# willake/cpu-ray-tracer

Hardware: AMD Instinct MI355X
Metric: Mrays/sec (primary+secondary), 1280x720 64spp path trace — pipelined throughput over 878 consecutive 64-spp windows of one progressive render (single_render = one such render alone) (higher is better)
Workload: dtype f32; 1 GPU; bunny_scene.xml FileScene BVH-SAH path tracer, 1280x720, 64 spp/step (passes=1, depthLimit=5); 1 step = 64 frames = the next spp window of a progressive render; the 878 steps are one crt_render job (14 render kernel launch(es), a wavefront per (tile, 128 consecutive frames), + ordered accumulate), one sync at the end; triangles=4968, parallelism=tile-wave x1

## Files before the change

cpu-ray-tracer_amd/csrc/abi.cpp:

```cpp
#include "../../include/crt_abi.h"
#include "device/launch.h"
#include "host/grid_resolution.h"

#include <cmath>
#include <cstdarg>
#include <cstddef>
#include <cstdio>
#include <cstdlib>
#include <cstring>
#include <deque>
#include <string>
#include <algorithm>
#include <vector>
#include <chrono>

static_assert(sizeof(crt_bvh_node) == 32 && sizeof(crt_tri) == 112 && sizeof(crt_tlas_node) == 32, "reference layouts");
static_assert(sizeof(crt::NodePair) == 64 && sizeof(crt::LeafTri) == 48 && sizeof(crt::ShadeTri) == 64 && sizeof(crt::TlasNode) == 32 &&
              sizeof(crt::Instance) == 128 && sizeof(crt::Material) == 32 && offsetof(crt::Instance, T) == 64, "device layouts");
static_assert(sizeof(crt_counters) == sizeof(crt::Counters), "counter layout");
static_assert(sizeof(crt_kd_node) == 48 && sizeof(crt::KdNode) == sizeof(crt_kd_node) && sizeof(crt::AltTri) == 48, "flat KD node (uploaded as it comes), alternative accelerators' triangle record");
static_assert(offsetof(crt::PrimDev, red) == 536 && sizeof(crt::PrimDev) == 552, "PrimDev: 134 floats, then the two texel pointers");
static_assert(sizeof(crt::BlasAltDesc) == 72, "BLAS descriptor");
static_assert(sizeof(crt_shadow_ray) == 28 && sizeof(crt_ray) == 28 && sizeof(crt_hit) == 28, "query records");
static_assert(sizeof(crt_hit_info) == 48 && offsetof(crt_hit_info, material) == 12 && offsetof(crt_hit_info, N) == 16 && offsetof(crt_hit_info, albedo) == 32 && offsetof(crt_hit_info, v) == 44, "crt_hit_info: three 16-byte pieces");
// ... 221 lines not shown
}

}

extern "C" {

int crt_abi_version(void) { return CRT_ABI_VERSION; }

void crt_debug_enable_hooks(int on) { g_hooks = on != 0; }

int crt_device_count(void)
{
    int n = 0;
    if (hipGetDeviceCount(&n) != hipSuccess) return 0;
    return n;
}

const char* crt_last_error(crt_ctx* ctx) { return ctx ? ctx->err.c_str() : g_createError.c_str(); }

int crt_create(crt_ctx** out, const crt_config* cfg)
{
    if (!out || !cfg) { g_createError = "crt_create: null argument"; return CRT_ERR_INVALID; }
    *out = nullptr;
    setenv("GPU_MAX_HW_QUEUES", "16", 0);
    if (cfg->width < 16 || cfg->height < 16) { g_createError = "crt_create: width and height must be at least one 16x16 tile"; return CRT_ERR_INVALID; }
    int ndev = 0;
    hipError_t e = hipGetDeviceCount(&ndev);
    if (e != hipSuccess || ndev == 0) {
        g_createError = "crt_create: no HIP device visible (this library has no CPU path)";
        return CRT_ERR_NO_DEVICE;
    }
    if (cfg->device < 0 || cfg->device >= ndev) { g_createError = "crt_create: device ordinal out of range"; return CRT_ERR_INVALID; }
    crt_ctx* c = new crt_ctx();
    c->cfg = *cfg;
    if (const char* k = hook("CRT_RENDER_KERNEL")) {
        c->usePool = strcmp(k, "tiles") != 0;
        if (!strcmp(k, "pool_always")) c->poolMinWaves = 0;
    }
    if (c->cfg.depthLimit < 0) c->cfg.depthLimit = 5;
    if (c->cfg.depthLimit > 5) { g_createError = "crt_create: depthLimit > 5 unsupported (throughput stack holds 5 factors; reference default is 5)"; delete c; return CRT_ERR_UNSUPPORTED; }
    if (c->cfg.maxFramesPerLaunch <= 0) c->cfg.maxFramesPerLaunch = c->cfg.collectStats ? 64 : 4096;
    if (c->cfg.maxFramesPerLaunch > 64) c->cfg.maxFramesPerLaunch = c->cfg.maxFramesPerLaunch / 64 * 64;
    if (c->cfg.renderStreams < 0) c->cfg.renderStreams = 0;
    c->tilesX = cfg->width / 16; c->tilesY = cfg->height / 16;
    const int tiles = c->tilesX * c->tilesY;
    int first = cfg->tileFirst, stride = cfg->tileStride <= 0 ? 1 : cfg->tileStride, count = cfg->tileCount;
    if (count < 0) { first = 0; stride = 1; count = tiles; }
    if (first < 0 || (count > 0 && (long long)first + (long long)(count - 1) * stride >= tiles)) {
        g_createError = "crt_create: tile range exceeds the image"; delete c; return CRT_ERR_INVALID;
    }
    c->tileFirst = (uint32_t)first; c->tileStride = (uint32_t)stride; c->tileCount = (uint32_t)count;

    auto bail = [&](hipError_t he, const char* what) {
        g_createError = std::string("crt_create: ") + what + ": " + hipGetErrorString(he);
        crt_destroy(c); return CRT_ERR_DEVICE;
    };
    if ((e = hipSetDevice(cfg->device)) != hipSuccess) return bail(e, "hipSetDevice");
    if ((e = hipStreamCreateWithFlags(&c->stream, hipStreamNonBlocking)) != hipSuccess) return bail(e, "hipStreamCreate");
    const size_t px = (size_t)cfg->width * cfg->height;
    if ((e = hipMalloc(&c->dAccOwned, px * 16)) != hipSuccess) return bail(e, "hipMalloc(accumulator)");
    c->dAcc = c->dAccOwned;
    if ((e = hipMemsetAsync(c->dAcc, 0, px * 16, c->stream)) != hipSuccess) return bail(e, "hipMemset(accumulator)");
    if ((e = hipMalloc((void**)&c->dPixels, px * 4)) != hipSuccess) return bail(e, "hipMalloc(pixels)");
    if ((e = hipMemsetAsync(c->dPixels, 0, px * 4, c->stream)) != hipSuccess) return bail(e, "hipMemset(pixels)");
    if ((e = hipMalloc((void**)&c->dTileSums, (size_t)tiles * 4)) != hipSuccess) return bail(e, "hipMalloc(tileSums)");
    if ((e = hipMemsetAsync(c->dTileSums, 0, (size_t)tiles * 4, c->stream)) != hipSuccess) return bail(e, "hipMemset(tileSums)");
    if ((e = hipMalloc((void**)&c->dCounters, sizeof(crt::Counters))) != hipSuccess) return bail(e, "hipMalloc(counters)");
    if ((e = hipMemsetAsync(c->dCounters, 0, sizeof(crt::Counters), c->stream)) != hipSuccess) return bail(e, "hipMemset(counters)");
    if ((e = hipMalloc((void**)&c->dQueryCursor, 64)) != hipSuccess) return bail(e, "hipMalloc(query cursor)");
    if ((e = hipMalloc((void**)&c->dQuerySlots, crt_ctx::kQuerySlots * 64)) != hipSuccess) return bail(e, "hipMalloc(query cursor slots)");
    if (c->cfg.collectStats && count > 0) {
        if ((e = hipMalloc((void**)&c->dTileClocks, (size_t)count * 144)) != hipSuccess) return bail(e, "hipMalloc(tileClocks)");
        if ((e = hipMemsetAsync(c->dTileClocks, 0, (size_t)count * 144, c->stream)) != hipSuccess) return bail(e, "hipMemset(tileClocks)");
    }
    memset(&c->hScene, 0, sizeof(c->hScene));
    const float aspect = (float)cfg->width / (float)cfg->height;
    crt::Scene& s = c->hScene;
    s.camPos[0] = 0; s.camPos[1] = 0; s.camPos[2] = -2;
    s.topLeft[0] = -aspect; s.topLeft[1] = 1; s.topLeft[2] = 0;
    s.topRight[0] = aspect; s.topRight[1] = 1; s.topRight[2] = 0;
    s.bottomLeft[0] = -aspect; s.bottomLeft[1] = -1; s.bottomLeft[2] = 0;
    s.W = cfg->width; s.H = cfg->height; s.invW = 1.0f / cfg->width; s.invH = 1.0f / cfg->height;
    s.depthLimit = c->cfg.depthLimit;
    if ((e = hipStreamSynchronize(c->stream)) != hipSuccess) return bail(e, "hipStreamSynchronize");
    *out = c;
    return CRT_OK;
}

void crt_destroy(crt_ctx* c)
{
    if (!c) return;
    (void)hipSetDevice(c->cfg.device);
    for (auto st : c->streams) (void)hipStreamSynchronize(st);
    if (c->aheadStream) (void)hipStreamSynchronize(c->aheadStream);
    if (c->stream) (void)hipStreamSynchronize(c->stream);
    for (auto& q : c->qslot) if (q.done) { if (q.pending) (void)hipEventSynchronize(q.done); (void)hipEventDestroy(q.done); }
    if (c->dQuerySlots) (void)hipFree(c->dQuerySlots);
    if (c->altReady) (void)hipEventDestroy(c->altReady);
    if (c->writeFence) (void)hipEventDestroy(c->writeFence);
    c->refit.release(); c->tlasBuild.release();
    c->freeScene();
    c->gridBuild.release();
    for (hipEvent_t e : c->retiredEvents) (void)hipEventDestroy(e);
    for (auto& a : c->ahead) (void)hipEventDestroy(a.end);
    if (c->aheadStream) (void)hipStreamDestroy(c->aheadStream);
    for (auto& ev : c->evPool) { (void)hipEventDestroy(ev.a); (void)hipEventDestroy(ev.b); }
    for (auto& ev : c->evRender) { (void)hipEventDestroy(ev.a); (void)hipEventDestroy(ev.b); }
    for (auto& ev : c->evAcc) { (void)hipEventDestroy(ev.a); (void)hipEventDestroy(ev.b); }
    if (c->dAccOwned) (void)hipFree(c->dAccOwned);
    for (auto st : c->streams) { (void)hipStreamSynchronize(st); (void)hipStreamDestroy(st); }
    for (auto& r : c->inflight) (void)hipEventDestroy(r.freed);
    for (auto e : c->freeEvents) (void)hipEventDestroy(e);
    if (c->mustWait) (void)hipEventDestroy(c->mustWait);
    if (c->pool) (void)hipFree(c->pool);
    for (auto e : c->doneEvents) (void)hipEventDestroy(e);
    if (c->dPixels) (void)hipFree(c->dPixels);
    if (c->dTileSums) (void)hipFree(c->dTileSums);
    if (c->dCounters) (void)hipFree(c->dCounters);
    if (c->dQueryCursor) (void)hipFree(c->dQueryCursor);
    if (c->dInspectCounts) (void)hipFree(c->dInspectCounts);
    if (c->dInspectWork) (void)hipFree(c->dInspectWork);
    if (c->dTileClocks) (void)hipFree(c->dTileClocks);
    if (c->dTileOrder) (void)hipFree(c->dTileOrder);
    if (c->dTileCost) (void)hipFree(c->dTileCost);
    if (c->dJobCost) (void)hipFree(c->dJobCost);
    if (c->dJobDesc) (void)hipFree(c->dJobDesc);
    if (c->hJobDesc) (void)hipHostFree(c->hJobDesc);
    if (c->jobDescReady) (void)hipEventDestroy(c->jobDescReady);
    if (c->hJobCost) (void)hipHostFree(c->hJobCost);
    if (c->jobCostCopied) (void)hipEventDestroy(c->jobCostCopied);
    for (auto e : c->splitEvents) (void)hipEventDestroy(e);
    if (c->hTileCost) (void)hipHostFree(c->hTileCost);
    if (c->costCopied) (void)hipEventDestroy(c->costCopied);
    if (c->dBlockDesc) (void)hipFree(c->dBlockDesc);
    if (c->hBlockDesc) (void)hipHostFree(c->hBlockDesc);
    if (c->descReady) (void)hipEventDestroy(c->descReady);
    if (c->dStage) (void)hipFree(c->dStage);
    for (int k = 0; k < 2; k++) { if (c->hTileOrder[k]) (void)hipHostFree(c->hTileOrder[k]); if (c->orderCopied[k]) (void)hipEventDestroy(c->orderCopied[k]); }
    for (int k = 0; k < 2; k++) { if (c->hStage[k]) (void)hipHostFree(c->hStage[k]); if (c->stageCopied[k]) (void)hipEventDestroy(c->stageCopied[k]); }
    if (c->stream) (void)hipStreamDestroy(c->stream);
    delete c;
}

int crt_upload_scene(crt_ctx* c, const crt_scene_desc* sd)
{
    if (!c || !sd) return CRT_ERR_INVALID;
    c->epoch++;
    HIPCK(c, hipSetDevice(c->cfg.device));
    if (sd->kind != CRT_SCENE_FILE && sd->kind != CRT_SCENE_TLAS) return c->fail(CRT_ERR_INVALID, "unknown scene kind %d", sd->kind);
    if (!sd->bvhs || sd->bvhCount == 0) return c->fail(CRT_ERR_INVALID, "scene has no acceleration structure");
    if (sd->kind == CRT_SCENE_FILE && sd->bvhCount != 1) return c->fail(CRT_ERR_INVALID, "CRT_SCENE_FILE takes exactly one BVH (FileScene::acc)");
    if (sd->kind == CRT_SCENE_TLAS && (sd->bvhCount > 256 || !sd->tlasNodes || sd->tlasNodeCount < 2 * sd->bvhCount))
        return c->fail(CRT_ERR_INVALID, "TLAS scene needs <= 256 BLAS (tlas_bvh.cpp:21) and 2*blasCount TLAS nodes");
    if (sd->textureCount == 0 || !sd->textures) return c->fail(CRT_ERR_INVALID, "floor and skydome textures are required");
    if (sd->floorTexture < 0 || sd->floorTexture >= (int)sd->textureCount || sd->skyTexture < 0 || sd->skyTexture >= (int)sd->textureCount)
        return c->fail(CRT_ERR_INVALID, "floor/sky texture index out of range");
    for (uint32_t i = 0; i < sd->textureCount; i++)
        if (!sd->textures[i].pixels || sd->textures[i].width <= 0 || sd->textures[i].height <= 0) return c->fail(CRT_ERR_INVALID, "texture %u is empty", i);
    if (sd->materialCount > 0 && !sd->materials) return c->fail(CRT_ERR_INVALID, "materialCount is %u but materials is NULL", sd->materialCount);
    for (uint32_t i = 0; i < sd->materialCount; i++)
        if (sd->materials[i].texture >= (int)sd->textureCount) return c->fail(CRT_ERR_INVALID, "material %u: texture index out of range", i);
    if (sd->kind == CRT_SCENE_FILE) {
        if (!sd->objMatIdx || sd->objCount == 0) return c->fail(CRT_ERR_INVALID, "CRT_SCENE_FILE needs objMatIdx");
        for (uint32_t i = 0; i < sd->objCount; i++)
            if (sd->objMatIdx[i] < 0 || sd->objMatIdx[i] >= (int)sd->materialCount) return c->fail(CRT_ERR_INVALID, "objMatIdx entry out of range");
    }
// ... 127 lines not shown
        }
        tlasRoot = tlas[0].ref; tlasRoot16 = tlas[0].ref16;
    }
    std::vector<uint32_t> texOff(sd->textureCount); uint64_t texels = 0;
    for (uint32_t i = 0; i < sd->textureCount; i++) {
        texOff[i] = (uint32_t)texels;
        texels += (uint64_t)sd->textures[i].width * sd->textures[i].height;
        if (texels > 0xffffffffull) return c->fail(CRT_ERR_UNSUPPORTED, "texture pool exceeds 2^32 texels");
    }
    auto bindTex = [&](crt::Material& m, int t) {
        if (t < 0) { m.texOffset = 0; m.texW = 0; m.texH = 0; }
        else { m.texOffset = texOff[t]; m.texW = sd->textures[t].width; m.texH = sd->textures[t].height; }
    };
    std::vector<crt::Material> mats(2 + sd->materialCount);
    memset(mats.data(), 0, mats.size() * sizeof(crt::Material));
    bindTex(mats[0], -1);
    bindTex(mats[1], sd->floorTexture);
    for (uint32_t i = 0; i < sd->materialCount; i++) {
        crt::Material& m = mats[2 + i];
        m.reflectivity = sd->materials[i].reflectivity; m.refractivity = sd->materials[i].refractivity;
        memcpy(m.absorption, sd->materials[i].absorption, 12);
        bindTex(m, sd->materials[i].texture);
    }

    { const int r = drain_all(c); if (r) return r; }
    c->freeScene();
    uint32_t* dTexels = nullptr;
    HIPCK(c, hipMalloc((void**)&dTexels, (size_t)texels * 4)); c->sceneAllocs.push_back(dTexels);
    for (uint32_t i = 0; i < sd->textureCount; i++)
        HIPCK(c, hipMemcpyAsync(dTexels + texOff[i], sd->textures[i].pixels, (size_t)sd->textures[i].width * sd->textures[i].height * 4, hipMemcpyHostToDevice, c->stream));
    HIPCK(c, hipStreamSynchronize(c->stream));

    crt::Scene& s = c->hScene;
    s.kind = sd->kind;
    memcpy(s.lightInvT, sd->lightInvT, 48);
    s.lightNrm[0] = -sd->lightT[1]; s.lightNrm[1] = -sd->lightT[5]; s.lightNrm[2] = -sd->lightT[9];
    s.lightSize = sd->lightSize;
    {
        const float* m = sd->lightT;
        const float ax = -0.5f, ay = 0.0f, az = -0.5f, bx = 0.5f, by = 0.0f, bz = 0.5f;
        const float c1[3] = {m[0] * ax + m[1] * ay + m[2] * az + m[3] * 1.0f, m[4] * ax + m[5] * ay + m[6] * az + m[7] * 1.0f, m[8] * ax + m[9] * ay + m[10] * az + m[11] * 1.0f};
        const float c2[3] = {m[0] * bx + m[1] * by + m[2] * bz + m[3] * 1.0f, m[4] * bx + m[5] * by + m[6] * bz + m[7] * 1.0f, m[8] * bx + m[9] * by + m[10] * bz + m[11] * 1.0f};
        s.lightPos[0] = (c1[0] + c2[0]) * 0.5f - 0.0f; s.lightPos[1] = (c1[1] + c2[1]) * 0.5f - 0.01f; s.lightPos[2] = (c1[2] + c2[2]) * 0.5f - 0.0f;
    }
    memcpy(s.floorN, sd->floorN, 12); s.floorD = sd->floorD; s.floorInvto = sd->floorInvto;
    {
        const float* m = sd->lightInvT;
        s.lightAxis = (m[0] == 1.0f && m[1] == 0.0f && m[2] == 0.0f && m[4] == 0.0f && m[5] == 1.0f && m[6] == 0.0f && m[8] == 0.0f && m[9] == 0.0f && m[10] == 1.0f) ? 1u : 0u;
        s.floorAxisY = (sd->floorN[0] == 0.0f && sd->floorN[1] == 1.0f && sd->floorN[2] == 0.0f) ? 1u : 0u;
        if (hook("CRT_DEBUG_GENERAL_PRIMS")) s.lightAxis = s.floorAxisY = 0u;
    }
    s.floorMat = mats[1];
    s.skyOffset = texOff[sd->skyTexture]; s.skyW = sd->textures[sd->skyTexture].width; s.skyH = sd->textures[sd->skyTexture].height;
    s.texels = dTexels;
    int r;
    const char* dGeom = nullptr;
    if ((r = upload(c, geom, &dGeom))) return r;
    s.geom = dGeom;
    s.tlasOff = (uint32_t)tlasOffB; s.instOff = (uint32_t)instOffB; s.shadeOff = (uint32_t)shadeOffB;
    s.leafOff = (uint32_t)leafOffB; s.tlasPairOff = (uint32_t)tlasPairOffB;
    s.rootRef16 = (sd->kind == CRT_SCENE_TLAS) ? tlasRoot16 : rootRef0_16;
    s.ref16ok = (ref16ok && !hook("CRT_DEBUG_NO_REF16")) ? 1u : 0u;
    if ((r = upload(c, mats, &s.mats))) return r;
    if (sd->kind == CRT_SCENE_TLAS) {
        std::vector<float> boxes;
        for (uint32_t bi = 0; bi < sd->bvhCount; bi++) { const crt_bvh_node& n0 = sd->bvhs[bi].nodes[0]; boxes.insert(boxes.end(), n0.aabbMin, n0.aabbMin + 3); boxes.insert(boxes.end(), n0.aabbMax, n0.aabbMax + 3); }
        const float* d = nullptr;
        if ((r = upload(c, boxes, &d))) return r;
        c->dRootBox = const_cast<float*>(d);
    }
    s.rootRef = (sd->kind == CRT_SCENE_TLAS) ? tlasRoot : rootRef0;
    s.bvhStack = maxHeight > 0 ? maxHeight : 1;
    s.rootIsPair = 0; memset(s.rootPair, 0, sizeof(s.rootPair));
    if (sd->kind == CRT_SCENE_TLAS) {
        if ((tlasRoot & 0xC0000000u) == crt::kRefTlasInterior) {
            memcpy(s.rootPair, &tlas[tlasRoot & 0x7fffu], 32); memcpy(s.rootPair + 8, &tlas[(tlasRoot >> 15) & 0x7fffu], 32);
            s.rootIsPair = 1;
        }
    } else if (rootRef0 & crt::kRefInterior) {
        memcpy(s.rootPair, geom.data() + ((size_t)(rootRef0 & crt::kRefOffsetMask) << 4), 64);
        s.rootIsPair = 1;
    }
    if (hook("CRT_DEBUG_NO_ROOTPAIR")) s.rootIsPair = 0;
    s.stackDepth = s.bvhStack + ((sd->kind == CRT_SCENE_TLAS) ? tlasHeight + 1 : 0);
    c->ldsBytes = s.stackDepth * 64u * 4u; c->latSlots = 0;
    if (const char* e = hook("CRT_DEBUG_EXTRA_LDS")) c->ldsBytes += (uint32_t)atoi(e);
    if (c->ldsBytes + 15u * 256u > 64u * 1024u) return c->fail(CRT_ERR_UNSUPPORTED, "tree height %u (+TLAS %u) needs %u bytes of LDS traversal stack per wave (> 64 KiB)", maxHeight, tlasHeight, c->ldsBytes);
    {
        float lo[3] = {1e30f, 1e30f, 1e30f}, hi[3] = {-1e30f, -1e30f, -1e30f};
        auto grow = [&](const float* mn, const float* mx) { for (int k = 0; k < 3; k++) { if (mn[k] < lo[k]) lo[k] = mn[k]; if (mx[k] > hi[k]) hi[k] = mx[k]; } };
        if (sd->kind == CRT_SCENE_TLAS) grow(sd->tlasNodes[0].aabbMin, sd->tlasNodes[0].aabbMax);
        else grow(sd->bvhs[0].nodes[0].aabbMin, sd->bvhs[0].nodes[0].aabbMax);
        memcpy(c->meshLo, lo, 12); memcpy(c->meshHi, hi, 12); c->orderDirty = true;
    }
    {
        crt_ctx::Flat& f = c->flat;
        f.kind = sd->kind; f.leafOff = leafOffB; f.tlasOff = tlasOffB; f.tlasPairOff = tlasPairOffB; f.instOff = instOffB; f.shadeOff = shadeOffB;
        f.tlasNodeCount = (sd->kind == CRT_SCENE_TLAS) ? sd->tlasNodeCount : 0; f.maxHeight = maxHeight;
        f.objects = (sd->kind == CRT_SCENE_TLAS) ? sd->bvhCount : sd->objCount;
        f.pairBase.clear(); f.triBase.clear(); f.nodesUsed.clear(); f.triCount.clear(); f.rootBox.clear();
        for (uint32_t bi = 0; bi < sd->bvhCount; bi++) { const crt_bvh_node& r = sd->bvhs[bi].nodes[0]; f.rootBox.insert(f.rootBox.end(), r.aabbMin, r.aabbMin + 3); f.rootBox.insert(f.rootBox.end(), r.aabbMax, r.aabbMax + 3); }
        uint64_t pb = 0, tb = 0;
        for (uint32_t bi = 0; bi < sd->bvhCount; bi++) { f.pairBase.push_back(pb); f.triBase.push_back(tb); f.nodesUsed.push_back(sd->bvhs[bi].nodesUsed); f.triCount.push_back(sd->bvhs[bi].triCount); pb += sd->bvhs[bi].nodesUsed / 2; tb += sd->bvhs[bi].triCount; }
        f.geom.swap(geom);
    }
    c->haveScene = true;
    return CRT_OK;
}


static int order_behind_ahead(crt_ctx* c)
{
    for (const auto& a : c->ahead) HIPCK(c, hipStreamWaitEvent(c->stream, a.end, 0));
    return 0;
}

static int order_behind_queries(crt_ctx* c)
{
    for (auto& q : c->qslot) {
        if (!q.pending) continue;
        const hipError_t e = hipEventQuery(q.done);
        if (e == hipSuccess) { q.pending = false; continue; }
        if (e != hipErrorNotReady) return c->hip(e, "hipEventQuery(query)");
        HIPCK(c, hipStreamWaitEvent(c->stream, q.done, 0));
    }
    return 0;
}

static int wait_scene(crt_ctx* c, hipStream_t st)
{
    if (c->sceneReady) HIPCK(c, hipStreamWaitEvent(st, c->sceneReady, 0));
    return 0;
}

static int order_behind_readers(crt_ctx* c)
{
    int r;
    if ((r = order_behind_ahead(c)) || (r = order_behind_queries(c))) return r;
    c->epoch++;
    return 0;
}

static int begin_scene_write(crt_ctx* c, hipStream_t st)
{
    const int r = order_behind_readers(c);
    if (r || st == c->stream) return r;
    HIPCK(c, ensure_event(&c->writeFence));
    HIPCK(c, hipEventRecord(c->writeFence, c->stream));
    HIPCK(c, hipStreamWaitEvent(st, c->writeFence, 0));
    return wait_scene(c, st);
}

static int publish_scene_write(crt_ctx* c, hipStream_t st, hipEvent_t done)
{
    c->sceneReady = done;
    if (st != c->stream) HIPCK(c, hipStreamWaitEvent(c->stream, done, 0));
    return 0;
}

static int end_scene_write(crt_ctx* c, hipStream_t st, hipEvent_t done)
{
    HIPCK(c, hipEventRecord(done, st));
    return publish_scene_write(c, st, done);
}

static int flatten_tlas(crt_ctx* c, const crt_tlas_node* nodes, uint32_t count, uint32_t bvhCount, crt::TlasNode* tlas, crt::NodePair* tlasPairs, uint32_t* heightOut)
{
    uint32_t nTlasPairs = 0;
    for (uint32_t i = 0; i < count; i++) {
        const crt_tlas_node& nd = nodes[i];
        memcpy(tlas[i].lo, nd.aabbMin, 12); memcpy(tlas[i].hi, nd.aabbMax, 12);
        tlas[i].ref = nd.leftRight ? (crt::kRefTlasInterior | (nd.leftRight & 0x7fffu) | (((nd.leftRight >> 16) & 0x7fffu) << 15))
                                   : (crt::kRefTlasLeaf | (nd.BLAS & 0xffffu));
        tlas[i].ref16 = nd.leftRight ? (crt::kRef16TlasBit | nTlasPairs++) : (crt::kRef16TlasLeaf | (nd.BLAS & crt::kRef16IndexMask));
    }
    std::vector<std::pair<uint32_t, uint32_t>> st; st.push_back({0u, 0u}); size_t visited = 0; uint32_t height = 0;
    while (!st.empty()) {
        auto [n, d] = st.back(); st.pop_back();
        if (++visited > (size_t)count) return c->fail(CRT_ERR_INVALID, "TLAS node graph is not a tree");
        const crt_tlas_node& nd = nodes[n];
        if (nd.leftRight == 0) { if (nd.BLAS >= bvhCount) return c->fail(CRT_ERR_INVALID, "TLAS leaf references BLAS %u", nd.BLAS); if (d > height) height = d; continue; }
        const uint32_t l = nd.leftRight & 0xffffu, r = nd.leftRight >> 16;
        if (l >= count || r >= count) return c->fail(CRT_ERR_INVALID, "TLAS child index out of range");
        st.push_back({l, d + 1}); st.push_back({r, d + 1});
    }
    for (uint32_t i = 0; i < count; i++) {
        const crt_tlas_node& nd = nodes[i];
        if (nd.leftRight == 0) continue;
        crt::NodePair& p = tlasPairs[tlas[i].ref16 & crt::kRef16IndexMask];
        memcpy(&p.c[0], &tlas[nd.leftRight & 0xffffu], 32); memcpy(&p.c[1], &tlas[nd.leftRight >> 16], 32);
    }
    *heightOut = height;
    return 0;
}

static void set_root(crt_ctx* c, int kind, const float* lo, const float* hi)
{
    crt::Scene& s = c->hScene; const crt_ctx::Flat& f = c->flat;
    s.rootIsPair = 0; memset(s.rootPair, 0, sizeof(s.rootPair));
    if (kind == CRT_SCENE_TLAS) {
        const crt::TlasNode* tlas = reinterpret_cast<const crt::TlasNode*>(f.geom.data() + f.tlasOff);
        const uint32_t root = tlas[0].ref;
        s.rootRef = root; s.rootRef16 = tlas[0].ref16;
        if ((root & 0xC0000000u) == crt::kRefTlasInterior) { memcpy(s.rootPair, &tlas[root & 0x7fffu], 32); memcpy(s.rootPair + 8, &tlas[(root >> 15) & 0x7fffu], 32); s.rootIsPair = 1; }
    } else if (s.rootRef & crt::kRefInterior) {
        memcpy(s.rootPair, f.geom.data() + ((size_t)(s.rootRef & crt::kRefOffsetMask) << 4), 64);
        s.rootIsPair = 1;
    }
    if (hook("CRT_DEBUG_NO_ROOTPAIR")) s.rootIsPair = 0;
    memcpy(c->meshLo, lo, 12); memcpy(c->meshHi, hi, 12); c->orderDirty = true;
}

static int check_tlas_height(crt_ctx* c, uint32_t tlasHeight)
{
    if ((c->hScene.bvhStack + tlasHeight + 1) * 64u * 4u + 15u * 256u > 64u * 1024u)
        return c->fail(CRT_ERR_UNSUPPORTED, "TLAS height %u needs %u bytes of LDS traversal stack per wave (> 64 KiB)", tlasHeight, (c->hScene.bvhStack + tlasHeight + 1) * 256u);
    return 0;
}

static void adopt_tlas(crt_ctx* c, uint32_t tlasHeight, const float* lo, const float* hi)
{
    crt::Scene& s = c->hScene;
    s.stackDepth = s.bvhStack + tlasHeight + 1;
    c->ldsBytes = s.stackDepth * 64u * 4u; c->latSlots = 0;
    set_root(c, CRT_SCENE_TLAS, lo, hi);
}

static void drop_blas_sets(crt_ctx* c)
{
    for (int k = 0; k < 2; k++) if (c->haveBlas[k]) { c->haveBlas[k] = false; if (c->renderAccel == k + 1) c->renderAccel = 0; }
}

int crt_update_scene(crt_ctx* c, const crt_scene_desc* sd, uint32_t what)
{
    if (!c || !sd) return CRT_ERR_INVALID;
    if (!c->haveScene) return c->fail(CRT_ERR_STATE, "crt_update_scene before crt_upload_scene");
    crt_ctx::Flat& f = c->flat;
    if (sd->kind != f.kind || sd->bvhCount != f.nodesUsed.size() || !sd->bvhs) return c->fail(CRT_ERR_INVALID, "crt_update_scene: scene kind / BVH count differ from the uploaded scene");
    if ((what & ~(uint32_t)(CRT_UPDATE_TRANSFORMS | CRT_UPDATE_BOUNDS)) || what == 0) return c->fail(CRT_ERR_INVALID, "crt_update_scene: unknown update flags");
    if ((what & CRT_UPDATE_TRANSFORMS) && f.kind != CRT_SCENE_TLAS) return c->fail(CRT_ERR_INVALID, "CRT_UPDATE_TRANSFORMS applies to two-level scenes (a FileScene bakes its transforms into the triangles)");
    HIPCK(c, hipSetDevice(c->cfg.device));
    for (uint32_t bi = 0; bi < sd->bvhCount; bi++)
        if (sd->bvhs[bi].nodesUsed != f.nodesUsed[bi] || sd->bvhs[bi].triCount != f.triCount[bi] || !sd->bvhs[bi].nodes || !sd->bvhs[bi].triangles || !sd->bvhs[bi].triangleIndices)
            return c->fail(CRT_ERR_INVALID, "crt_update_scene: BVH %u changed its topology (node / triangle count); upload the scene again", bi);
    if (f.kind == CRT_SCENE_TLAS && (!sd->tlasNodes || sd->tlasNodeCount != f.tlasNodeCount))
        return c->fail(CRT_ERR_INVALID, "crt_update_scene: a two-level scene needs the node array of the TLASBVH::Build that followed the change (tlasNodes, %u nodes as uploaded)", f.tlasNodeCount);
    if (what & CRT_UPDATE_BOUNDS) {
        const crt::LeafTri* leaf = reinterpret_cast<const crt::LeafTri*>(f.geom.data() + f.leafOff);
        for (uint32_t bi = 0; bi < sd->bvhCount; bi++) {
            const crt_bvh& b = sd->bvhs[bi];
            for (uint32_t j = 0; j < b.triCount; j++) {
                const uint32_t ti = b.triangleIndices[j];
                if (ti >= b.triCount) return c->fail(CRT_ERR_INVALID, "BVH %u: triangleIndices[%u] out of range", bi, j);
                if (leaf[f.triBase[bi] + j].shadeIdx != (uint32_t)(f.triBase[bi] + ti)) return c->fail(CRT_ERR_INVALID, "BVH %u: triangleIndices changed; Refit keeps the leaf order — upload the scene again", bi);
            }
        }
    }
    uint32_t tlasHeight = 0;
    std::vector<char> tlasImage;
    if (f.kind == CRT_SCENE_TLAS) {
        tlasImage.assign((size_t)(f.instOff - f.tlasOff), 0);
        int r = flatten_tlas(c, sd->tlasNodes, sd->tlasNodeCount, sd->bvhCount, reinterpret_cast<crt::TlasNode*>(tlasImage.data()),
                             reinterpret_cast<crt::NodePair*>(tlasImage.data() + (f.tlasPairOff - f.tlasOff)), &tlasHeight);
        if (r || (r = check_tlas_height(c, tlasHeight))) return r;
    }
    size_t lo = SIZE_MAX, hi = 0;
    auto touch = [&](size_t a, size_t b) { if (a < lo) lo = a; if (b > hi) hi = b; };
    if (what & CRT_UPDATE_BOUNDS) {
        crt::NodePair* pairs = reinterpret_cast<crt::NodePair*>(f.geom.data());
        crt::LeafTri* leaf = reinterpret_cast<crt::LeafTri*>(f.geom.data() + f.leafOff);
        for (uint32_t bi = 0; bi < sd->bvhCount; bi++) {
            const crt_bvh& b = sd->bvhs[bi];
            for (uint32_t n = 1; n + 1 < b.nodesUsed; n += 2) {
                crt::NodePair& p = pairs[f.pairBase[bi] + ((n - 1) >> 1)];
                for (int k = 0; k < 2; k++) { memcpy(p.c[k].lo, b.nodes[n + k].aabbMin, 12); memcpy(p.c[k].hi, b.nodes[n + k].aabbMax, 12); }
            }
            for (uint32_t j = 0; j < b.triCount; j++) {
                const crt_tri& t = b.triangles[b.triangleIndices[j]];
                crt::LeafTri& lt = leaf[f.triBase[bi] + j];
                for (int k = 0; k < 3; k++) { lt.v0[k] = t.vertex0[k]; lt.e1[k] = t.vertex1[k] - t.vertex0[k]; lt.e2[k] = t.vertex2[k] - t.vertex0[k]; }
            }
        }
        touch(0, (size_t)f.tlasOff);
        for (uint32_t bi = 0; bi < sd->bvhCount; bi++) { memcpy(&f.rootBox[6 * bi], sd->bvhs[bi].nodes[0].aabbMin, 12); memcpy(&f.rootBox[6 * bi + 3], sd->bvhs[bi].nodes[0].aabbMax, 12); }
    }
    if (f.kind == CRT_SCENE_TLAS) {
        if (what & CRT_UPDATE_TRANSFORMS) {
            crt::Instance* inst = reinterpret_cast<crt::Instance*>(f.geom.data() + f.instOff);
            for (uint32_t bi = 0; bi < sd->bvhCount; bi++) { memcpy(inst[bi].invT, sd->bvhs[bi].invT, 48); memcpy(inst[bi].T, sd->bvhs[bi].T, 48); }
        }
        memcpy(f.geom.data() + f.tlasOff, tlasImage.data(), tlasImage.size());
        touch((size_t)f.tlasOff, (size_t)f.shadeOff);
    }
    if (lo >= hi) return CRT_OK;
    const int k = c->stageFlip ^= 1;
    const size_t boxBytes = ((what & CRT_UPDATE_BOUNDS) && c->dRootBox) ? f.rootBox.size() * 4u : 0u;
    const size_t geomBytes = hi - lo, bytes = geomBytes + boxBytes;
    if (c->stageBytes[k] < bytes) {
        if (c->hStage[k]) { HIPCK(c, hipEventSynchronize(c->stageCopied[k])); HIPCK(c, hipHostFree(c->hStage[k])); c->hStage[k] = nullptr; }
        HIPCK(c, hipHostMalloc((void**)&c->hStage[k], bytes, hipHostMallocDefault)); c->stageBytes[k] = bytes;
        HIPCK(c, ensure_event(&c->stageCopied[k]));
    } else HIPCK(c, hipEventSynchronize(c->stageCopied[k]));
    memcpy(c->hStage[k], f.geom.data() + lo, geomBytes);
    if (boxBytes) memcpy(c->hStage[k] + geomBytes, f.rootBox.data(), boxBytes);
    { const int r = begin_scene_write(c, c->stream); if (r) return r; }
    if (what & CRT_UPDATE_BOUNDS) {
        std::fill(c->blasGrid.current.begin(), c->blasGrid.current.end(), (uint8_t)0);
        drop_blas_sets(c);
    }
    HIPCK(c, hipMemcpyAsync(const_cast<char*>(c->hScene.geom) + lo, c->hStage[k], geomBytes, hipMemcpyHostToDevice, c->stream));
    if (boxBytes) HIPCK(c, hipMemcpyAsync(c->dRootBox, c->hStage[k] + geomBytes, boxBytes, hipMemcpyHostToDevice, c->stream));
    { const int r = end_scene_write(c, c->stream, c->stageCopied[k]); if (r) return r; }
    if (f.kind == CRT_SCENE_TLAS) adopt_tlas(c, tlasHeight, sd->tlasNodes[0].aabbMin, sd->tlasNodes[0].aabbMax);
    else set_root(c, f.kind, sd->bvhs[0].nodes[0].aabbMin, sd->bvhs[0].nodes[0].aabbMax);
    return CRT_OK;
}

int crt_set_camera(crt_ctx* c, const float camPos[3], const float tl[3], const float tr[3], const float bl[3])
{
    if (!c || !camPos || !tl || !tr || !bl) return CRT_ERR_INVALID;
    HIPCK(c, hipSetDevice(c->cfg.device));
    crt::Scene& s = c->hScene;
    if (!memcmp(s.camPos, camPos, 12) && !memcmp(s.topLeft, tl, 12) && !memcmp(s.topRight, tr, 12) && !memcmp(s.bottomLeft, bl, 12)) return CRT_OK;
    memcpy(s.camPos, camPos, 12); memcpy(s.topLeft, tl, 12); memcpy(s.topRight, tr, 12); memcpy(s.bottomLeft, bl, 12);
    c->orderDirty = true; c->epoch++;
    return CRT_OK;
}

static int upload_tile_order(crt_ctx* c, const std::vector<uint32_t>& order)
{
    if (!c->dTileOrder) HIPCK(c, hipMalloc((void**)&c->dTileOrder, (size_t)c->tileCount * 4));
    { const int r = order_behind_ahead(c); if (r) return r; }
    const int k = c->orderFlip ^= 1;
    if (!c->hTileOrder[k]) {
        HIPCK(c, hipHostMalloc((void**)&c->hTileOrder[k], (size_t)c->tileCount * 4, hipHostMallocDefault));
        HIPCK(c, ensure_event(&c->orderCopied[k]));
    } else HIPCK(c, hipEventSynchronize(c->orderCopied[k]));
    memcpy(c->hTileOrder[k], order.data(), order.size() * 4);
    HIPCK(c, hipMemcpyAsync(c->dTileOrder, c->hTileOrder[k], order.size() * 4, hipMemcpyHostToDevice, c->stream));
    HIPCK(c, hipEventRecord(c->orderCopied[k], c->stream));
    c->orderReady = c->orderCopied[k];
    return 0;
}

static int update_tile_order(crt_ctx* c)
{
    if (!c->orderDirty || c->tileCount == 0) return 0;
    const crt::Scene& s = c->hScene;
    double R[3], Dn[3], N[3];
    for (int k = 0; k < 3; k++) { R[k] = (double)s.topRight[k] - s.topLeft[k]; Dn[k] = (double)s.bottomLeft[k] - s.topLeft[k]; }
    N[0] = R[1] * Dn[2] - R[2] * Dn[1]; N[1] = R[2] * Dn[0] - R[0] * Dn[2]; N[2] = R[0] * Dn[1] - R[1] * Dn[0];
    const double rr = R[0] * R[0] + R[1] * R[1] + R[2] * R[2], dd = Dn[0] * Dn[0] + Dn[1] * Dn[1] + Dn[2] * Dn[2];
    double E[3]; for (int k = 0; k < 3; k++) E[k] = (double)s.topLeft[k] - s.camPos[k];
    const double num = E[0] * N[0] + E[1] * N[1] + E[2] * N[2];
    auto rect_of = [&](const float* P8, int r[4]) -> bool {
        double u0 = 1e30, u1 = -1e30, v0 = 1e30, v1 = -1e30;
        for (int i = 0; i < 8; i++) {
            const float* P = P8 + 3 * i;
            double d[3] = {P[0] - s.camPos[0], P[1] - s.camPos[1], P[2] - s.camPos[2]};
            const double den = d[0] * N[0] + d[1] * N[1] + d[2] * N[2];
            const double t = den != 0 ? num / den : -1;
            if (!(t > 0) || rr == 0 || dd == 0) return false;
            double Q[3]; for (int k = 0; k < 3; k++) Q[k] = s.camPos[k] + t * d[k] - s.topLeft[k];
            const double u = (Q[0] * R[0] + Q[1] * R[1] + Q[2] * R[2]) / rr, v = (Q[0] * Dn[0] + Q[1] * Dn[1] + Q[2] * Dn[2]) / dd;
            if (u < u0) u0 = u; if (u > u1) u1 = u; if (v < v0) v0 = v; if (v > v1) v1 = v;
        }
        r[0] = (int)floor(u0 * c->cfg.width / 16.0) - 1; r[1] = (int)floor(u1 * c->cfg.width / 16.0) + 1;
        r[2] = (int)floor(v0 * c->cfg.height / 16.0) - 1; r[3] = (int)floor(v1 * c->cfg.height / 16.0) + 1;
        return true;
    };
    float world[24];
    for (int i = 0; i < 8; i++) { world[3 * i] = (i & 1) ? c->meshHi[0] : c->meshLo[0]; world[3 * i + 1] = (i & 2) ? c->meshHi[1] : c->meshLo[1]; world[3 * i + 2] = (i & 4) ? c->meshHi[2] : c->meshLo[2]; }
    int wr[4] = {0, c->tilesX - 1, 0, c->tilesY - 1};
    (void)rect_of(world, wr);
    std::vector<uint32_t> first, second, rest;
    for (uint32_t i = 0; i < c->tileCount; i++) {
        const uint32_t tile = c->tileFirst + i * c->tileStride;
        const int tx = (int)(tile % (uint32_t)c->tilesX), ty = (int)(tile / (uint32_t)c->tilesX);
        const bool inRect = tx >= wr[0] && tx <= wr[1] && ty >= wr[2] && ty <= wr[3];
        if (inRect) first.push_back(i); else rest.push_back(i);
    }
    for (int k = 0; k <= crt_ctx::kLatStages; k++) { c->tuneCount[k] = 0; c->tuneMs[k] = 0; }
    c->latStage = 0; c->latBest = 0; c->latDone = false; c->latWarm = false; c->latConfirming = false; c->latQueue.clear(); c->costPending = false; c->latProbed = false;
    first.insert(first.end(), rest.begin(), rest.end());
    c->jobCostValid = false; c->jobCostPending = false; c->planValid = false;
    { const int r = upload_tile_order(c, first); if (r) return r; }
    c->orderDirty = false;
    return 0;
}

static size_t sample_bytes_per_window(const crt_ctx* c, uint32_t passes) { return (size_t)c->tileCount * 256u * 64u * passes * 16u; }
static size_t window_bytes(const crt_ctx* c, uint32_t passes) { return sample_bytes_per_window(c, passes) + (c->usePool ? crt_pool_scratch_bytes_per_window(c->tileCount) : 0); }

static uint32_t block_desc(uint32_t tile, uint32_t laneBase, uint32_t lanes, uint32_t window) { uint32_t lg = 0; while ((1u << lg) < lanes) lg++; return tile | (laneBase << 16) | (lg << 22) | (window << 25); }
static const uint32_t kLatLanes[7] = {64u, 32u, 16u, 8u, 4u, 2u, 1u};
static const double kLatG[7] = {1.0, 0.93, 0.88, 0.79, 0.69, 0.57, 0.48};
static int lat_index(uint32_t L) { int k = 0; while (k < 6 && kLatLanes[k] != L) k++; return k; }

static uint8_t next_lanes(uint8_t lanes, uint32_t cost, double T)
{
    int k = lat_index(lanes); const double unit = (double)cost / kLatG[k];
    while (k < 6 && unit * kLatG[k] > T) k++;
    while (k > 0 && unit * kLatG[k - 1] <= 0.9 * T) k--;
    return (uint8_t)kLatLanes[k];
}
extern "C" int crt_debug_next_lanes(const uint8_t* lanes, const uint32_t* cost, uint32_t n, double T, uint8_t* out)
{
// ... 1685 lines not shown
{
    if (!c || !out) return CRT_ERR_INVALID;
    int r;
    if ((r = sample_check(c, accel, 0, "crt_debug_sample_resident_lanes"))) return r;
    HIPCK(c, hipSetDevice(c->cfg.device));
    HIPCK(c, launch_sample(c, accel, nullptr, nullptr, nullptr, 0u, nullptr, out, c->stream));
    return CRT_OK;
}

int crt_get_light(crt_ctx* c, float pos[3], float color[3])
{
    if (!c || !pos || !color) return CRT_ERR_INVALID;
    if (!c->haveScene) return c->fail(c->havePrim ? CRT_ERR_UNSUPPORTED : CRT_ERR_STATE, "crt_get_light needs a triangle scene (crt_upload_scene)");
    memcpy(pos, c->hScene.lightPos, 12);
    color[0] = 24.0f; color[1] = 24.0f; color[2] = 22.0f;
    return CRT_OK;
}

int crt_get_counters(crt_ctx* c, crt_counters* out)
{
    if (!c || !out) return CRT_ERR_INVALID;
    HIPCK(c, hipSetDevice(c->cfg.device));
    HIPCK(c, hipMemcpyAsync(out, c->dCounters, sizeof(crt::Counters), hipMemcpyDeviceToHost, c->stream));
    HIPCK(c, hipStreamSynchronize(c->stream));
    return CRT_OK;
}

int crt_reset_counters(crt_ctx* c)
{
    if (!c) return CRT_ERR_INVALID;
    HIPCK(c, hipSetDevice(c->cfg.device));
    HIPCK(c, hipMemsetAsync(c->dCounters, 0, sizeof(crt::Counters), c->stream));
    return CRT_OK;
}

int crt_get_timing(crt_ctx* c, crt_timing* out)
{
    if (!c || !out) return CRT_ERR_INVALID;
    HIPCK(c, hipSetDevice(c->cfg.device));
    HIPCK(c, hipStreamSynchronize(c->stream));
    for (auto st : c->streams) HIPCK(c, hipStreamSynchronize(st));
    if (c->aheadStream) HIPCK(c, hipStreamSynchronize(c->aheadStream));
    harvest_tuning(c);
    memset(out, 0, sizeof(*out));
    out->render_kernel_ms = (float)c->foldedRenderMs; out->resolve_kernel_ms = (float)c->foldedAccMs;
    for (auto& ev : c->evRender) { float ms = 0; HIPCK(c, hipEventElapsedTime(&ms, ev.a, ev.b)); out->render_kernel_ms += ms; }
    for (auto& ev : c->evAcc) { float ms = 0; HIPCK(c, hipEventElapsedTime(&ms, ev.a, ev.b)); out->resolve_kernel_ms += ms; }
    out->render_launches = (uint32_t)c->evRender.size() + c->foldedLaunches;
    out->pool_launches = c->poolLaunches; out->split_launches = c->splitLaunches;
    c->foldedRenderMs = c->foldedAccMs = 0; c->foldedLaunches = 0; c->poolLaunches = 0; c->splitLaunches = 0;
    for (auto& ev : c->evRender) c->evPool.push_back(ev);
    for (auto& ev : c->evAcc) c->evPool.push_back(ev);
    c->evRender.clear(); c->evAcc.clear();
    return CRT_OK;
}

int crt_get_tile_clocks(crt_ctx* c, uint64_t* out)
{
    if (!c || !out) return CRT_ERR_INVALID;
    if (!c->dTileClocks) return c->fail(CRT_ERR_STATE, "tile clocks are recorded only by a collectStats context");
    HIPCK(c, hipSetDevice(c->cfg.device));
    HIPCK(c, hipMemcpyAsync(out, c->dTileClocks, (size_t)c->tileCount * 16, hipMemcpyDeviceToHost, c->stream));
    HIPCK(c, hipStreamSynchronize(c->stream));
    return CRT_OK;
}

extern "C" int crt_debug_live_events(crt_ctx* c) { return c ? (int)(2 * (c->evRender.size() + c->evAcc.size() + c->evPool.size())) : -1; }

extern "C" int crt_debug_check_reciprocals(crt_ctx* c, uint64_t* out)
{
    if (!c || !out) return CRT_ERR_INVALID;
    HIPCK(c, hipSetDevice(c->cfg.device));
    unsigned long long* d = nullptr;
    HIPCK(c, hipMalloc(&d, 32));
    hipError_t e = hipMemsetAsync(d, 0, 32, c->stream);
    if (e == hipSuccess) e = crt_launch_check_reciprocals(d, c->stream);
    if (e == hipSuccess) e = hipMemcpyAsync(out, d, 32, hipMemcpyDeviceToHost, c->stream);
    if (e == hipSuccess) e = hipStreamSynchronize(c->stream);
    (void)hipFree(d);
    HIPCK(c, e);
    return CRT_OK;
}

extern "C" int crt_debug_device_probe(crt_ctx* c, int op, const void* in, void* out, uint32_t n)
{
    static const uint8_t words[17][2] = {{1, 1}, {1, 1}, {2, 1}, {1, 1}, {2, 1}, {6, 7}, {1, 18}, {4, 1}, {5, 3}, {13, 2}, {16, 4}, {2, 2}, {2, 2}, {2, 2}, {2, 2}, {4, 2}, {2, 1}};
    if (!c || !in || !out || op < 0 || op > 16 || n > (1u << 25)) return CRT_ERR_INVALID;
    if (n == 0) return CRT_OK;
    const size_t inBytes = (size_t)n * words[op][0] * 4, outBytes = (size_t)n * words[op][1] * 4;
    HIPCK(c, hipSetDevice(c->cfg.device));
    char* d = nullptr;
    HIPCK(c, hipMalloc((void**)&d, inBytes + outBytes));
    hipError_t e = hipMemcpyAsync(d, in, inBytes, hipMemcpyHostToDevice, c->stream);
    if (e == hipSuccess) e = (op <= 10) ? crt_launch_probe_f32(op, d, d + inBytes, n, c->stream) : crt_launch_probe_f64(op, d, d + inBytes, n, c->stream);
    if (e == hipSuccess) e = hipMemcpyAsync(out, d + inBytes, outBytes, hipMemcpyDeviceToHost, c->stream);
    if (e == hipSuccess) e = hipStreamSynchronize(c->stream);
    (void)hipFree(d);
    HIPCK(c, e);
    return CRT_OK;
}

extern "C" int crt_debug_plan_job(const uint32_t* cost, uint32_t n, uint32_t windows, uint32_t frames, int pool, double poolWindowTicks,
                                  uint32_t* table, uint32_t tableCap, uint32_t* head, uint32_t* order)
{
    if (!cost || !n || !table || !head || !order) return CRT_ERR_INVALID;
    crt_ctx c;
    c.tileCount = n; c.jobCostValid = true; c.poolWindowTicks = poolWindowTicks;
    c.streams.assign(2, nullptr);
    c.jobCost.assign(cost, cost + n);
    c.jobOrder.resize(n);
    for (uint32_t i = 0; i < n; i++) c.jobOrder[i] = i;
    std::stable_sort(c.jobOrder.begin(), c.jobOrder.end(), [&](uint32_t a, uint32_t b) { return c.jobCost[a] > c.jobCost[b]; });
    std::vector<uint32_t> t; uint32_t h = 0;
    plan_job(&c, windows, frames, pool != 0, t, &h);
    c.streams.clear();
    if (t.size() > tableCap) return CRT_ERR_INVALID;
    memcpy(table, t.data(), t.size() * 4); memcpy(order, c.jobOrder.data(), (size_t)n * 4); *head = h;
    return (int)t.size();
}

extern "C" long long crt_debug_pool_wave_plan(const uint32_t* cost, uint32_t nr, uint32_t frames, double perCost, double startTicks, uint32_t resident, double safety, double guard,
                                              double share, uint32_t* wf, uint32_t* longFrames, double* start, double* aim)
{
    if (!nr || !frames || !wf || !longFrames) return CRT_ERR_INVALID;
    PoolWaveTerms tm; if (safety > 0) tm.safety = safety; if (guard > 0) tm.guard = guard; if (share > 0) tm.share = share;
    std::vector<uint32_t> w; std::vector<double> st;
    const uint64_t waves = pool_wave_plan(cost, nr, frames, crt_pool_streams(frames), perCost, startTicks, resident, tm, w, longFrames, &st, aim);
    memcpy(wf, w.data(), (size_t)nr * 4);
    if (start) memcpy(start, st.data(), (size_t)nr * 8);
    return (long long)waves;
}
extern "C" int crt_debug_pool_long_waves(crt_ctx* c) { return c ? (int)c->lastLongWaves : -1; }
extern "C" void crt_debug_pool_wave_terms(double* out) { const PoolWaveTerms tm; out[0] = tm.poolLong; out[1] = tm.load; out[2] = tm.safety; out[3] = tm.guard; out[4] = tm.share; }

extern "C" int crt_debug_tile_costs(crt_ctx* c, uint32_t* out)
{
    if (!c || !out || !c->dTileCost) return CRT_ERR_INVALID;
    HIPCK(c, hipSetDevice(c->cfg.device));
    HIPCK(c, hipDeviceSynchronize());
    HIPCK(c, hipMemcpy(out, c->dTileCost, (size_t)c->tileCount * 4, hipMemcpyDeviceToHost));
    return CRT_OK;
}

extern "C" int crt_debug_lat_stage(crt_ctx* c, int stage, uint8_t* lanes, uint32_t* cost)
{
    if (!c || stage < 0 || stage > crt_ctx::kLatStages) return CRT_ERR_INVALID;
    if (c->latL[stage].size() != c->tileCount || c->latCost[stage].size() != c->tileCount) return CRT_ERR_STATE;
    if (lanes) memcpy(lanes, c->latL[stage].data(), c->tileCount);
    if (cost) memcpy(cost, c->latCost[stage].data(), (size_t)c->tileCount * 4);
    return c->latStage;
}

extern "C" int crt_debug_tile_stamps(crt_ctx* c, uint64_t* out)
{
    if (!c || !out || !c->dTileClocks) return CRT_ERR_INVALID;
    HIPCK(c, hipSetDevice(c->cfg.device));
    HIPCK(c, hipMemcpyAsync(out, c->dTileClocks + 2 * (size_t)c->tileCount, (size_t)c->tileCount * 128, hipMemcpyDeviceToHost, c->stream));
    HIPCK(c, hipStreamSynchronize(c->stream));
    return CRT_OK;
}

int crt_bind_accumulator(crt_ctx* c, void* p)
{
    if (!c) return CRT_ERR_INVALID;
    if (p && ((uintptr_t)p & 15u)) return c->fail(CRT_ERR_INVALID, "accumulator pointer must be 16-byte aligned");
    HIPCK(c, hipSetDevice(c->cfg.device));
    HIPCK(c, hipStreamSynchronize(c->stream));
    c->dAcc = p ? p : c->dAccOwned;
    return CRT_OK;
}

int crt_accumulator_device_ptr(crt_ctx* c, void** p)
{
    if (!c || !p) return CRT_ERR_INVALID;
    *p = c->dAcc; return CRT_OK;
}

}
```

cpu-ray-tracer_amd/csrc/device/dev_common.h:

```cpp
#pragma once
#include <hip/hip_runtime.h>
#include <stddef.h>
#include <stdint.h>
#include "layout.h"

namespace crt {

struct f3 { float x, y, z; };
__device__ __forceinline__ f3 mk3(float x, float y, float z) { f3 r; r.x = x; r.y = y; r.z = z; return r; }
__device__ __forceinline__ f3 operator+(f3 a, f3 b) { return mk3(a.x + b.x, a.y + b.y, a.z + b.z); }
__device__ __forceinline__ f3 operator-(f3 a, f3 b) { return mk3(a.x - b.x, a.y - b.y, a.z - b.z); }
__device__ __forceinline__ f3 operator-(f3 a) { return mk3(-a.x, -a.y, -a.z); }
__device__ __forceinline__ f3 operator*(f3 a, f3 b) { return mk3(a.x * b.x, a.y * b.y, a.z * b.z); }
__device__ __forceinline__ f3 operator*(f3 a, float b) { return mk3(a.x * b, a.y * b, a.z * b); }
__device__ __forceinline__ f3 operator*(float b, f3 a) { return mk3(b * a.x, b * a.y, b * a.z); }
__device__ __forceinline__ float dot3(f3 a, f3 b) { return a.x * b.x + a.y * b.y + a.z * b.z; }
__device__ __forceinline__ f3 cross3(f3 a, f3 b) { return mk3(a.y * b.z - a.z * b.y, a.z * b.x - a.x * b.z, a.x * b.y - a.y * b.x); }
#ifdef CRT_IEEE_DIV
__device__ __forceinline__ float rcp_nr(float x) { return 1.0f / x; }
#else
__device__ __forceinline__ float rcp_nr(float x) { const float r = __builtin_amdgcn_rcpf(x); return __builtin_fmaf(__builtin_fmaf(-x, r, 1.0f), r, r); }
#endif
__device__ __forceinline__ float rcp_exact(float x)
{
    float r = rcp_nr(x);
    const float ax = __builtin_fabsf(x);
    if (__builtin_expect(__builtin_amdgcn_ballot_w64(!(ax >= 0x1p-126f && ax <= 0x1p126f)) != 0, 0)) r = 1.0f / x;
    return r;
}
__device__ __forceinline__ float rcp_exact_large(float x)
{
    float r = rcp_nr(x);
    if (__builtin_expect(__builtin_amdgcn_ballot_w64(!(__builtin_fabsf(x) <= 0x1p126f)) != 0, 0)) r = 1.0f / x;
    return r;
}
__device__ __forceinline__ f3 rcp_exact3(f3 v)
{
    f3 r = mk3(rcp_nr(v.x), rcp_nr(v.y), rcp_nr(v.z));
    const float ax = __builtin_fabsf(v.x), ay = __builtin_fabsf(v.y), az = __builtin_fabsf(v.z);
    const bool okay = ax >= 0x1p-126f && ay >= 0x1p-126f && az >= 0x1p-126f && ax <= 0x1p126f && ay <= 0x1p126f && az <= 0x1p126f;
    if (__builtin_expect(__builtin_amdgcn_ballot_w64(!okay) != 0, 0)) r = mk3(1.0f / v.x, 1.0f / v.y, 1.0f / v.z);
    return r;
}
__device__ __forceinline__ f3 normalize3(f3 v) { float inv = rcp_exact(__builtin_sqrtf(dot3(v, v))); return v * inv; }
__device__ __forceinline__ float min_std(float a, float b) { return (b < a) ? b : a; }
__device__ __forceinline__ float max_std(float a, float b) { return (a < b) ? b : a; }
__device__ __forceinline__ float min_tm(float a, float b) { return a < b ? a : b; }
__device__ __forceinline__ float max_tm(float a, float b) { return a > b ? a : b; }
__device__ __forceinline__ float clamp_tm(float f, float a, float b) { return max_tm(a, min_tm(f, b)); }
__device__ __forceinline__ int clampi(int f, int a, int b) { int m = (b < f) ? b : f; return (a < m) ? m : a; }
__device__ __forceinline__ float asf(uint32_t u) { return __uint_as_float(u); }
__device__ __forceinline__ uint32_t asu(float f) { return __float_as_uint(f); }

#define CRT_PI 3.14159265358979323846264f
#define CRT_INVPI 0.31830988618379067153777f
#define CRT_INV2PI 0.15915494309189533576888f
#define CRT_EPS 0.001f

static __device__ float crt_expf(float x)
{
    if (x != x) return x;
    if (x > 88.72283905206835f) return asf(0x7f800000u);
    if (x < -103.972084045410f) return 0.0f;
    float fk = __builtin_floorf(x * 1.44269504088896341f + 0.5f);
    float r = x - fk * 0.693359375f;
    r = r - fk * -2.12194440e-4f;
    float z = r * r;
    float p = 1.9875691500e-4f;
    p = p * r + 1.3981999507e-3f;
    p = p * r + 8.3334519073e-3f;
    p = p * r + 4.1665795894e-2f;
    p = p * r + 1.6666665459e-1f;
    p = p * r + 5.0000001201e-1f;
    p = p * z + r;
    p = p + 1.0f;
    int k = (int)fk;
    int k1 = k / 2, k2 = k - k1;
    float s1 = asf((uint32_t)(k1 + 127) << 23), s2 = asf((uint32_t)(k2 + 127) << 23);
    return p * s1 * s2;
}
__device__ __forceinline__ float crt_atan_pos(float x)
{
    const bool big = x > 2.414213562373095f, mid = x > 0.4142135623730950f;
    const float y0 = big ? 1.5707963267948966f : (mid ? 0.7853981633974483f : 0.0f);
    const float num = big ? -1.0f : (mid ? x - 1.0f : x);
    const float den = big ? x : (mid ? x + 1.0f : 1.0f);
    const float t = num / den;
    float z = t * t;
    float p = 8.05374449538e-2f;
    p = p * z - 1.38776856032e-1f;
    p = p * z + 1.99777106478e-1f;
    p = p * z - 3.33329491539e-1f;
    p = p * z * t + t;
    return y0 + p;
}
__device__ __forceinline__ float crt_atan2f(float y, float x)
{
    const uint32_t sy = asu(y) & 0x80000000u, sx = asu(x) & 0x80000000u;
    const float ax = __builtin_fabsf(x), ay = __builtin_fabsf(y);
    const float inf = asf(0x7f800000u);
    const float a = crt_atan_pos(ay / ax);
    float r = sx ? (CRT_PI - a) : a;
    if (ax == inf && ay == inf) r = sx ? 2.356194490192345f : 0.7853981633974483f;
    if (ax == 0.0f) r = 1.5707963267948966f;
    if (ay == 0.0f) r = sx ? CRT_PI : 0.0f;
    r = asf(asu(r) | sy);
    return (x != x || y != y) ? x + y : r;
}
__device__ __forceinline__ float crt_asin_small(float x)
{
    float z = x * x;
    float p = 4.2163199048e-2f;
    p = p * z + 2.4181311049e-2f;
    p = p * z + 4.5470025998e-2f;
    p = p * z + 7.4953002686e-2f;
    p = p * z + 1.6666752422e-1f;
    p = p * z * x + x;
    return p;
}
__device__ __forceinline__ float crt_acosf(float x)
{
    const bool hi = x > 0.5f, lo = x < -0.5f;
    const float s = __builtin_sqrtf(0.5f * (1.0f - __builtin_fabsf(x)));
    const float p = crt_asin_small((hi || lo) ? s : x);
    float r = hi ? 2.0f * p : (lo ? CRT_PI - 2.0f * p : 1.5707963267948966f - p);
    if (x > 1.0f || x < -1.0f) r = asf(0x7fc00000u);
    return (x != x) ? x : r;
}

__device__ __forceinline__ uint32_t wang_hash(uint32_t s)
{
    s = (s ^ 61u) ^ (s >> 16); s *= 9u; s = s ^ (s >> 4); s *= 0x27d4eb2du; s = s ^ (s >> 15); return s;
}
__device__ __forceinline__ uint32_t init_seed(uint32_t base) { return wang_hash((base + 1u) * 17u); }
__device__ __forceinline__ float rnd(uint32_t& s)
{
    s ^= s << 13; s ^= s >> 17; s ^= s << 5;
    return (float)s * 2.3283064365387e-10f;
}
__device__ __forceinline__ float rnd_pm1(uint32_t& s)
{
    s ^= s << 13; s ^= s >> 17; s ^= s << 5;
    return __builtin_fmaf((float)s, 4.656612873077392578125e-10f, -1.0f);
}


struct Hit { float t, u, v; int objIdx, triIdx; };
struct Cnt { uint32_t rays, primary, interior, leaf, tri, tlas, visits, meshhits; };

typedef float rec4 __attribute__((ext_vector_type(4)));
__device__ __forceinline__ rec4 ld4(const void* p) { return *reinterpret_cast<const rec4*>(p); }
__device__ __forceinline__ rec4 ldg(const char* __restrict__ base, uint32_t byteOff) { return *reinterpret_cast<const rec4*>(base + byteOff); }
__device__ __forceinline__ bool finite3(f3 v)
{
    const uint32_t m = 0x7f800000u;
    return ((asu(v.x) & m) != m) && ((asu(v.y) & m) != m) && ((asu(v.z) & m) != m);
}

__device__ __forceinline__ float box_exact(rec4 lo, rec4 hi, f3 O, f3 rD, float tray)
{
    float tx1 = (lo.x - O.x) * rD.x, tx2 = (hi.x - O.x) * rD.x;
    float tmin = min_std(tx1, tx2), tmax = max_std(tx1, tx2);
    float ty1 = (lo.y - O.y) * rD.y, ty2 = (hi.y - O.y) * rD.y;
    tmin = max_std(tmin, min_std(ty1, ty2)); tmax = min_std(tmax, max_std(ty1, ty2));
    float tz1 = (lo.z - O.z) * rD.z, tz2 = (hi.z - O.z) * rD.z;
    tmin = max_std(tmin, min_std(tz1, tz2)); tmax = min_std(tmax, max_std(tz1, tz2));
    return (tmax >= tmin && tmin < tray && tmax > 0) ? tmin : 1e30f;
}
__device__ __forceinline__ float vmin(float a, float b) { float r; asm("v_min_f32 %0, %1, %2" : "=v"(r) : "v"(a), "v"(b)); return r; }
__device__ __forceinline__ float vmax(float a, float b) { float r; asm("v_max_f32 %0, %1, %2" : "=v"(r) : "v"(a), "v"(b)); return r; }
__device__ __forceinline__ float vmin3(float a, float b, float c) { float r; asm("v_min3_f32 %0, %1, %2, %3" : "=v"(r) : "v"(a), "v"(b), "v"(c)); return r; }
__device__ __forceinline__ float vmax3(float a, float b, float c) { float r; asm("v_max3_f32 %0, %1, %2, %3" : "=v"(r) : "v"(a), "v"(b), "v"(c)); return r; }
__device__ __forceinline__ float box_fast(rec4 lo, rec4 hi, f3 O, f3 rD, float tray)
{
    float tx1 = (lo.x - O.x) * rD.x, tx2 = (hi.x - O.x) * rD.x;
    float ty1 = (lo.y - O.y) * rD.y, ty2 = (hi.y - O.y) * rD.y;
    float tz1 = (lo.z - O.z) * rD.z, tz2 = (hi.z - O.z) * rD.z;
    float tmin = vmax3(vmin(tx1, tx2), vmin(ty1, ty2), vmin(tz1, tz2));
    float tmax = vmin3(vmax(tx1, tx2), vmax(ty1, ty2), vmax(tz1, tz2));
    return (tmax >= tmin && tmin < tray && tmax > 0) ? tmin : 1e30f;
}

__device__ __forceinline__ void hit_tri(rec4 a, rec4 b, rec4 c, f3 O, f3 D, Hit& h)
{
    const f3 v0 = mk3(a.x, a.y, a.z), e1 = mk3(b.x, b.y, b.z), e2 = mk3(c.x, c.y, c.z);
    const f3 hh = cross3(D, e2);
    const float det = dot3(e1, hh);
    const float f = rcp_exact_large(det);
    const f3 s = O - v0;
    const float u = f * dot3(s, hh);
    const f3 q = cross3(s, e1);
    const float v = f * dot3(D, q);
    const float t = f * dot3(e2, q);
    const bool ok = !(det > -0.0001f && det < 0.0001f) && !(u < 0 || u > 1) && !(v < 0 || u + v > 1) && (t > 0.0001f) && (t < h.t);
    if (ok) { h.t = t; h.u = u; h.v = v; h.triIdx = (int)asu(a.w); h.objIdx = (int)asu(b.w); }
}

struct LightFloor { float lightInvT[12]; float lightSize; uint32_t lightAxis, floorAxisY; float floorN[3]; float floorD; };
__device__ __forceinline__ void hit_light_floor(const LightFloor& sc, f3 O, f3 D, Hit& h)
{
    {
        const float* c = sc.lightInvT;
        float Oy, Dy;
        if (sc.lightAxis) { Oy = O.y + c[7]; Dy = D.y; }
        else { Oy = c[4] * O.x + c[5] * O.y + c[6] * O.z + c[7]; Dy = c[4] * D.x + c[5] * D.y + c[6] * D.z; }
        const float t = Oy / -Dy;
        if (t < h.t && t > 0) {
            float Ox, Oz, Dx, Dz;
            if (sc.lightAxis) { Ox = O.x + c[3]; Oz = O.z + c[11]; Dx = D.x; Dz = D.z; }
            else {
                Ox = c[0] * O.x + c[1] * O.y + c[2] * O.z + c[3];
                Oz = c[8] * O.x + c[9] * O.y + c[10] * O.z + c[11];
                Dx = c[0] * D.x + c[1] * D.y + c[2] * D.z;
                Dz = c[8] * D.x + c[9] * D.y + c[10] * D.z;
            }
            const float Ix = Ox + t * Dx, Iz = Oz + t * Dz;
            const float size = sc.lightSize;
            if (Ix > -size && Ix < size && Iz > -size && Iz < size) { h.t = t; h.objIdx = 0; }
        }
    }
    {
        float num, den;
        if (sc.floorAxisY) { num = O.y + sc.floorD; den = D.y; }
        else { const f3 N = mk3(sc.floorN[0], sc.floorN[1], sc.floorN[2]); num = dot3(O, N) + sc.floorD; den = dot3(D, N); }
        const float t = -num / den;
        if (t < h.t && t > 0) { h.t = t; h.objIdx = 1; }
    }
}

__device__ __forceinline__ void hit_light_floor(const Scene& sc, f3 O, f3 D, Hit& h)
{
    LightFloor lf;
#pragma unroll
    for (int i = 0; i < 12; i++) lf.lightInvT[i] = sc.lightInvT[i];
    lf.lightSize = sc.lightSize; lf.lightAxis = sc.lightAxis; lf.floorAxisY = sc.floorAxisY;
    lf.floorN[0] = sc.floorN[0]; lf.floorN[1] = sc.floorN[1]; lf.floorN[2] = sc.floorN[2]; lf.floorD = sc.floorD;
    hit_light_floor(lf, O, D, h);
}

__device__ __forceinline__ bool quad_occluded(const Scene& sc, f3 O, f3 D, float tmax)
{
    const float* c = sc.lightInvT;
    const float Oy = c[4] * O.x + c[5] * O.y + c[6] * O.z + c[7];
    const float Dy = c[4] * D.x + c[5] * D.y + c[6] * D.z;
    const float t = Oy / -Dy;
    if (!(t < tmax && t > 0)) return false;
    const float Ox = c[0] * O.x + c[1] * O.y + c[2] * O.z + c[3];
    const float Oz = c[8] * O.x + c[9] * O.y + c[10] * O.z + c[11];
    const float Dx = c[0] * D.x + c[1] * D.y + c[2] * D.z;
    const float Dz = c[8] * D.x + c[9] * D.y + c[10] * D.z;
    const float Ix = Ox + t * Dx, Iz = Oz + t * Dz;
    const float size = sc.lightSize;
    return Ix > -size && Ix < size && Iz > -size && Iz < size;
}

static_assert(offsetof(Scene, topLeft) == offsetof(Scene, camPos) + 12 && offsetof(Scene, bottomLeft) == offsetof(Scene, camPos) + 36 && offsetof(Scene, invW) == offsetof(Scene, camPos) + 48 && offsetof(Scene, invH) == offsetof(Scene, camPos) + 52, "camera block");
static_assert(offsetof(Scene, lightSize) == offsetof(Scene, lightInvT) + 60 && offsetof(Scene, floorN) == offsetof(Scene, lightInvT) + 76 && offsetof(Scene, floorD) == offsetof(Scene, lightInvT) + 88 && offsetof(Scene, floorInvto) == offsetof(Scene, floorN) + 16, "light / floor block");
static_assert(offsetof(Scene, floorAxisY) == offsetof(Scene, lightAxis) + 4 && offsetof(Scene, skyW) == offsetof(Scene, skyOffset) + 4 && offsetof(Scene, skyH) == offsetof(Scene, skyOffset) + 8, "flag / sky words");
static_assert(offsetof(Material, absorption) == 8 && offsetof(Material, texOffset) == 20 && offsetof(Material, texW) == 24 && offsetof(Material, texH) == 28, "Material words");
typedef const float __attribute__((address_space(4)))* kernarg_f;
__device__ __forceinline__ kernarg_f scene_floats(size_t byteOffset)
{
    const char __attribute__((address_space(4)))* p = (const char __attribute__((address_space(4)))*)__builtin_amdgcn_kernarg_segment_ptr() + byteOffset;
    asm volatile("" : "+s"(p));
    return (kernarg_f)p;
}

__device__ __forceinline__ void to_object_space(rec4 r0, rec4 r1, rec4 r2, f3 O, f3 D, f3& Oo, f3& Do, f3& rDo)
{
    Oo = mk3((O.x * r0.x + O.y * r0.y) + (O.z * r0.z + 1.0f * r0.w),
             (O.x * r1.x + O.y * r1.y) + (O.z * r1.z + 1.0f * r1.w),
             (O.x * r2.x + O.y * r2.y) + (O.z * r2.z + 1.0f * r2.w));
    Do = mk3((D.x * r0.x + D.y * r0.y) + D.z * r0.z,
             (D.x * r1.x + D.y * r1.y) + D.z * r1.z,
             (D.x * r2.x + D.y * r2.y) + D.z * r2.z);
    rDo = rcp_exact3(Do);
}

__device__ __forceinline__ void traverse_bvh_seq(const Scene& sc, uint32_t rootRef, f3 O, f3 D, f3 rD, Hit& h, uint32_t* stk, Cnt& cn,
                                                 int& traversed, int& tested)
{
    const char* __restrict__ g = sc.geom;
    uint32_t cur = rootRef, sp = 0;
    for (;;) {
        traversed++;
        const uint32_t off = (cur & kRefOffsetMask) << 4;
        if (cur & kRefInterior) {
            cn.interior++;
            const rec4 alo = ldg(g, off), ahi = ldg(g, off + 16), blo = ldg(g, off + 32), bhi = ldg(g, off + 48);
            float d1 = box_exact(alo, ahi, O, rD, h.t), d2 = box_exact(blo, bhi, O, rD, h.t);
            uint32_t r1 = asu(alo.w), r2 = asu(blo.w);
            if (d1 > d2) { float td = d1; d1 = d2; d2 = td; uint32_t tr = r1; r1 = r2; r2 = tr; }
            if (d1 == 1e30f) { if (sp == 0) break; cur = stk[(--sp) * 64]; }
            else { cur = r1; if (d2 != 1e30f) { stk[sp * 64] = r2; sp++; } }
        } else {
            cn.leaf++;
            uint32_t o = off;
            for (;;) {
                const rec4 a = ldg(g, o), b = ldg(g, o + 16), c = ldg(g, o + 32);
                tested++; cn.tri++;
                hit_tri(a, b, c, O, D, h);
                if (asu(c.w) <= 1u) break;
                o += 48;
            }
            if (sp == 0) break;
            cur = stk[(--sp) * 64];
        }
    }
}

template <bool STOP = false, class BlasWalk>
__device__ __forceinline__ void tlas_walk(const Scene& sc, f3 O, f3 D, f3 rD, Hit& h, uint32_t* tstk, Cnt& cn, int& traversed, BlasWalk&& blas)
{
    const char* __restrict__ g = sc.geom;
    uint32_t cur = sc.rootRef, sp = 0;
    for (;;) {
        traversed++; cn.tlas++;
        if ((cur & kRefTlasLeaf) == kRefTlasLeaf) {
            cn.visits++;
            const uint32_t io = sc.instOff + (cur & 0xffffu) * 128u;
            const rec4 r0 = ldg(g, io), r1 = ldg(g, io + 16), r2 = ldg(g, io + 32), ids = ldg(g, io + 48);
            f3 Oo, Do, rDo; to_object_space(r0, r1, r2, O, D, Oo, Do, rDo);
            if constexpr (STOP) { if (blas(cur & 0xffffu, ids, Oo, Do, rDo)) break; }
            else blas(cur & 0xffffu, ids, Oo, Do, rDo);
            if (sp == 0) break;
            cur = tstk[(--sp) * 64];
        } else {
            const uint32_t o1 = sc.tlasOff + (cur & 0x7fffu) * 32u, o2 = sc.tlasOff + ((cur >> 15) & 0x7fffu) * 32u;
            const rec4 alo = ldg(g, o1), ahi = ldg(g, o1 + 16), blo = ldg(g, o2), bhi = ldg(g, o2 + 16);
            float d1 = box_exact(alo, ahi, O, rD, h.t), d2 = box_exact(blo, bhi, O, rD, h.t);
            uint32_t r1 = asu(alo.w), r2 = asu(blo.w);
            if (d1 > d2) { float td = d1; d1 = d2; d2 = td; uint32_t tr = r1; r1 = r2; r2 = tr; }
            if (d1 == 1e30f) { if (sp == 0) break; cur = tstk[(--sp) * 64]; }
            else { cur = r1; if (d2 != 1e30f) { tstk[sp * 64] = r2; sp++; } }
        }
    }
}

__device__ __forceinline__ void find_nearest_seq(const Scene& sc, f3 O, f3 D, f3 rD, Hit& h, uint32_t* stk, Cnt& cn, int& traversed, int& tested)
{
    cn.rays++;
    hit_light_floor(sc, O, D, h);
    if (sc.kind == 0) {
        traverse_bvh_seq(sc, sc.rootRef, O, D, rD, h, stk, cn, traversed, tested);
    } else {
        tlas_walk(sc, O, D, rD, h, stk + sc.bvhStack * 64, cn, traversed, [&](uint32_t, rec4 ids, f3 Oo, f3 Do, f3 rDo) __attribute__((always_inline)) {
            traverse_bvh_seq(sc, asu(ids.z), Oo, Do, rDo, h, stk, cn, traversed, tested);
        });
    }
    if (h.objIdx >= 2) cn.meshhits++;
}

__device__ __forceinline__ uint32_t tex_index(uint32_t offset, int w, int hgt, float u, float v)
{
    u = clamp_tm(u, 0.0f, 1.0f);
    v = 1 - clamp_tm(v, 0.0f, 1.0f);
    int x = (int)(u * w), y = (int)(v * hgt);
    x = clampi(x, 0, w - 1); y = clampi(y, 0, hgt - 1);
    return offset + (uint32_t)x + (uint32_t)y * (uint32_t)w;
}
__device__ __forceinline__ f3 tex_unpack(uint32_t p)
{
    const float s = 1 / 255.0f;
    return mk3(((p >> 16) & 0xFF) * s, ((p >> 8) & 0xFF) * s, (p & 0xFF) * s);
}
__device__ __forceinline__ f3 tex_sample(const Scene& sc, uint32_t offset, int w, int hgt, float u, float v)
{
    return tex_unpack(sc.texels[tex_index(offset, w, hgt, u, v)]);
}

__device__ __forceinline__ f3 sky_color(const Scene& sc, f3 D)
{
    float phi = crt_atan2f(-D.z, D.x) + CRT_PI;
    float theta = crt_acosf(-D.y);
    return tex_sample(sc, sc.skyOffset, sc.skyW, sc.skyH, phi * CRT_INV2PI, theta * CRT_INVPI);
}

__device__ __forceinline__ uint32_t wave_sum(uint32_t v)
{
    for (int o = 32; o > 0; o >>= 1) v += __shfl_xor(v, o, 64);
    return v;
}

}
```

cpu-ray-tracer_amd/csrc/device/kernels.hip:

```cpp
#include "alt_common.h"
#include "launch.h"

namespace crt {

#ifndef CRT_SHADE_BATCH
#define CRT_SHADE_BATCH 24
#endif
#ifndef CRT_SHADE_BATCH_JOB
#define CRT_SHADE_BATCH_JOB 40
#endif
#ifndef CRT_TRI_BATCH
#define CRT_TRI_BATCH 1
#endif
#ifndef CRT_NODE_BATCH
#define CRT_NODE_BATCH 1
#endif

#ifndef CRT_TILES_NODE_STEPS
#define CRT_TILES_NODE_STEPS 2
#endif
#ifndef CRT_MIN_WAVES
#define CRT_MIN_WAVES 5
#endif
template <int KIND, bool COUNT>
// ... 939 lines not shown
    const int32_t before = __shfl_up(incl, 1, 64);
    if (lane > 0 && before > peak) peak = before;
    if (idx < n && pixels[idx] == kInspectPending) {
        const f3 res = traverse_count_color(own, peak);
        acc[idx] = make_float4(res.x, res.y, res.z, 0.0f);
        const uint32_t r = (uint32_t)(255.0f * min_std(1.0f, res.x)), g = (uint32_t)(255.0f * min_std(1.0f, res.y)), bb = (uint32_t)(255.0f * min_std(1.0f, res.z));
        pixels[idx] = (r << 16) + (g << 8) + bb;
    }
}

__global__ __launch_bounds__(64) void resolve_kernel(const float4* __restrict__ acc, uint32_t* __restrict__ pixels, float* __restrict__ tileSums,
                                                      uint32_t tileFirst, uint32_t tileStride, uint32_t tileCount, uint32_t tilesX,
                                                      uint32_t W, float scale)
{
    const uint32_t tl = blockIdx.x * blockDim.x + threadIdx.x;
    if (tl >= tileCount) return;
    const uint32_t tile = tileFirst + tl * tileStride;
    const uint32_t x0 = (tile % tilesX) * 16u, y0 = (tile / tilesX) * 16u;
    float sum = 0;
    for (uint32_t v = 0; v < 16; v++) for (uint32_t u = 0; u < 16; u++) {
        const size_t i = (x0 + u) + (size_t)(y0 + v) * W;
        const float4 a = acc[i];
        const float px = a.x * scale, py = a.y * scale, pz = a.z * scale;
        sum += px + py + pz;
        const uint32_t r = (uint32_t)(255.0f * min_std(1.0f, px)), g = (uint32_t)(255.0f * min_std(1.0f, py)), bb = (uint32_t)(255.0f * min_std(1.0f, pz));
        pixels[i] = (r << 16) + (g << 8) + bb;
    }
    tileSums[tile] = sum;
}

__global__ __launch_bounds__(256) void commit_frame_kernel(const float4* __restrict__ slabWindow, uint32_t frameInWindow, uint32_t passes,
                                                            float4* __restrict__ acc, uint32_t* __restrict__ pixels, float* __restrict__ tileSums,
                                                            uint32_t tileFirst, uint32_t tileStride, uint32_t tileCount, uint32_t tilesX,
                                                            uint32_t W, float scale)
{
    __shared__ float tileE[256];
    const uint32_t tl = blockIdx.x, pix = threadIdx.x;
    if (tl >= tileCount) return;
    const uint32_t tile = tileFirst + tl * tileStride;
    const uint32_t x0 = (tile % tilesX) * 16u, y0 = (tile / tilesX) * 16u;
    const size_t i = (x0 + (pix & 15u)) + (size_t)(y0 + (pix >> 4)) * W;
    const float4* __restrict__ s = slabWindow + ((size_t)tl * 256u + pix) * (64u * passes) + frameInWindow * passes;
    float4 a = acc[i];
    for (uint32_t p = 0; p < passes; p++) { const float4 t = s[p]; a.x += t.x; a.y += t.y; a.z += t.z; a.w += t.w; }
    acc[i] = a;
    const float px = a.x * scale, py = a.y * scale, pz = a.z * scale;
    tileE[pix] = px + py + pz;
    const uint32_t r = (uint32_t)(255.0f * min_std(1.0f, px)), g = (uint32_t)(255.0f * min_std(1.0f, py)), bb = (uint32_t)(255.0f * min_std(1.0f, pz));
    pixels[i] = (r << 16) + (g << 8) + bb;
    __syncthreads();
    if (pix == 0) {
        float sum = 0;
        for (uint32_t k = 0; k < 256u; k++) sum += tileE[k];
        tileSums[tile] = sum;
    }
}

}

namespace crt {
__device__ __forceinline__ bool same_bits(float a, float b) { return asu(a) == asu(b) || (a != a && b != b); }
__global__ __launch_bounds__(256) void check_reciprocals_kernel(unsigned long long* out)
{
    const uint32_t tid = blockIdx.x * 256u + threadIdx.x, nthreads = gridDim.x * 256u;
    unsigned long long n = 0, bad1 = 0, bad2 = 0, bad3 = 0;
    for (uint64_t b = tid; b < (1ull << 32); b += nthreads) {
        const float x = asf((uint32_t)b), want = 1.0f / x;
        n++;
        if (!same_bits(rcp_exact(x), want)) bad1++;
        if (!(__builtin_fabsf(x) < 0.0001f) && !same_bits(rcp_exact_large(x), want)) bad2++;
        const float y = asf((uint32_t)b * 2654435761u), z = asf(((uint32_t)b >> 7) * 40503u + 0x3f000000u);
        const f3 r = rcp_exact3(mk3(x, y, z));
        if (!same_bits(r.x, want) || !same_bits(r.y, 1.0f / y) || !same_bits(r.z, 1.0f / z)) bad3++;
    }
    atomicAdd(&out[0], n); atomicAdd(&out[1], bad1); atomicAdd(&out[2], bad2); atomicAdd(&out[3], bad3);
}
}
extern "C" hipError_t crt_launch_check_reciprocals(unsigned long long* out, hipStream_t stream)
{
    hipLaunchKernelGGL(crt::check_reciprocals_kernel, dim3(4096), dim3(256), 0, stream, out);
    return hipGetLastError();
}

extern "C" hipError_t crt_launch_render(const crt::Scene* sc, void* slab, crt::Counters* counters, unsigned long long* tileClocks, const uint32_t* tileOrder,
                                        uint32_t tileFirst, uint32_t tileStride, uint32_t tileCount, uint32_t tilesX, uint32_t sppFirst,
                                        uint32_t frames, uint32_t passes, uint32_t ldsBytes, int collectStats, const uint32_t* blockDesc, uint32_t nBlocks, uint32_t* tileCost, uint32_t rankCount, unsigned long long* launchClk, hipStream_t stream)
{
    if (tileCount == 0 || frames == 0) return hipSuccess;
    const uint32_t windows = (frames + 63u) / 64u;
    if ((unsigned long long)tileCount * windows > 0x7fffffffull) return hipErrorInvalidValue;
    if (collectStats || nBlocks == 0u) blockDesc = nullptr;
    if (blockDesc && (tileCount > 0x10000u || windows > 64u)) return hipErrorInvalidValue;
    if (rankCount == 0u || rankCount > tileCount) rankCount = tileCount;
    dim3 grid(blockDesc ? nBlocks : rankCount * windows), block(64);
#define CRT_LAUNCH(K, C) hipLaunchKernelGGL((crt::render_tiles_kernel<K, C>), grid, block, ldsBytes + 15u * 64u * 4u , stream, *sc, (float4*)slab, counters, tileClocks, tileOrder, tileFirst, tileStride, tileCount, tilesX, sppFirst, frames, passes, windows, blockDesc, tileCost, rankCount, launchClk)
    if (sc->kind == 0) { if (collectStats) CRT_LAUNCH(0, true); else CRT_LAUNCH(0, false); }
    else { if (collectStats) CRT_LAUNCH(1, true); else CRT_LAUNCH(1, false); }
#undef CRT_LAUNCH
    return hipGetLastError();
}

extern "C" uint32_t crt_render_resident_waves(int device, int kind, uint32_t ldsBytes)
{
    int perCu = 0, cus = 0;
    const size_t lds = (size_t)ldsBytes + 15u * 64u * 4u;
    hipError_t e = kind == 0 ? hipOccupancyMaxActiveBlocksPerMultiprocessor(&perCu, crt::render_tiles_kernel<0, false>, 64, lds)
                             : hipOccupancyMaxActiveBlocksPerMultiprocessor(&perCu, crt::render_tiles_kernel<1, false>, 64, lds);
    if (e != hipSuccess || hipDeviceGetAttribute(&cus, hipDeviceAttributeMultiprocessorCount, device) != hipSuccess || perCu <= 0 || cus <= 0) { (void)hipGetLastError(); return 5120u; }
    return (uint32_t)perCu * (uint32_t)cus;
}

extern "C" hipError_t crt_launch_accumulate(const void* slab, void* acc, uint32_t tileFirst, uint32_t tileStride, uint32_t tileCount,
                                            uint32_t tilesX, uint32_t W, uint32_t frames, uint32_t passes, hipStream_t stream)
{
    if (tileCount == 0 || frames == 0) return hipSuccess;
    dim3 grid(tileCount), block(256);
    hipLaunchKernelGGL(crt::accumulate_kernel, grid, block, 4u * crt::kAccWaveLds, stream, (const float4*)slab, (float*)acc, tileFirst, tileStride, tileCount, tilesX, W, frames, passes);
    return hipGetLastError();
}

extern "C" hipError_t crt_launch_find_nearest(const crt::Scene* sc, const void* rays, void* hits, uint32_t n, crt::Counters* counters,
                                              uint32_t ldsBytes, uint32_t* cursor, hipStream_t stream)
{
    hipError_t e; if (!crt::query_launch_begin(n, cursor, stream, &e)) return e;
    dim3 grid(crt::query_grid(n, ldsBytes)), block(64);
    hipLaunchKernelGGL(crt::find_nearest_kernel, grid, block, ldsBytes, stream, *sc, (const crt::RayIn*)rays, (crt::HitOut*)hits, n, counters, cursor);
    return hipGetLastError();
}

extern "C" hipError_t crt_launch_is_occluded(const crt::Scene* sc, const void* rays, int32_t* occluded, uint32_t n, uint32_t ldsBytes, uint32_t* cursor, hipStream_t stream)
{
    hipError_t e; if (!crt::query_launch_begin(n, cursor, stream, &e)) return e;
    dim3 grid(crt::query_grid(n, ldsBytes)), block(64);
    hipLaunchKernelGGL(crt::is_occluded_kernel, grid, block, ldsBytes, stream, *sc, (const crt::ShadowRayIn*)rays, occluded, n, cursor);
    return hipGetLastError();
}

extern "C" hipError_t crt_launch_whitted(const crt::Scene* sc, int accel, const crt::AltAccelDev* alt, const crt::TlasAltDev* tl, void* acc, uint32_t* pixels, crt::Counters* counters, uint32_t ldsBytes,
                                         hipStream_t stream)
{
    const uint32_t n = (uint32_t)sc->W * (uint32_t)sc->H;
    dim3 grid((n + 63u) / 64u), block(64);
    if (accel != 0 && sc->kind != 0) {
        const uint32_t bytes = crt::tlas_alt_stack_words(*sc, *tl) * 64u * 4u;
        if (bytes > 64u * 1024u) return hipErrorInvalidValue;
        if (accel == 1) hipLaunchKernelGGL((crt::whitted_kernel<1, crt::TlasAltDev>), grid, block, bytes, stream, *sc, *tl, (float4*)acc, pixels, counters);
        else hipLaunchKernelGGL((crt::whitted_kernel<2, crt::TlasAltDev>), grid, block, bytes, stream, *sc, *tl, (float4*)acc, pixels, counters);
        return hipGetLastError();
    }
    if (accel == 1) hipLaunchKernelGGL(crt::whitted_kernel<1>, grid, block, alt->kdStack * 128u * 4u, stream, *sc, *alt, (float4*)acc, pixels, counters);
    else if (accel == 2) hipLaunchKernelGGL(crt::whitted_kernel<2>, grid, block, 256u, stream, *sc, *alt, (float4*)acc, pixels, counters);
    else { const crt::AltAccelDev none{}; hipLaunchKernelGGL(crt::whitted_kernel<0>, grid, block, ldsBytes, stream, *sc, none, (float4*)acc, pixels, counters); }
    return hipGetLastError();
}

template <int ACCEL, class ALT>
static hipError_t launch_whitted_inspect(const crt::Scene& sc, const ALT& alt, uint32_t ldsBytes, int inspect, int32_t peakIn, float4* acc, uint32_t* pixels, crt::Counters* counters,
                                         int32_t* trav, int32_t* tested, crt::InspectSums* sums, int32_t* blockMax, hipStream_t stream)
{
    const uint32_t n = (uint32_t)sc.W * (uint32_t)sc.H;
    dim3 grid((n + 63u) / 64u), block(64);
    if (inspect == 0) {
        const crt::InspectOut out{trav, tested, sums};
        hipLaunchKernelGGL((crt::whitted_kernel<ACCEL, ALT, crt::InspectOut>), grid, block, ldsBytes, stream, sc, alt, acc, pixels, counters, out);
        return hipGetLastError();
    }
// ... 52 lines not shown
```

cpu-ray-tracer_amd/csrc/device/launch.h:

```cpp
#pragma once
#include "layout.h"

#include <hip/hip_runtime.h>

extern "C" {

hipError_t crt_launch_check_reciprocals(unsigned long long* out, hipStream_t stream);
hipError_t crt_launch_render(const crt::Scene* sc, void* slab, crt::Counters* counters, unsigned long long* tileClocks, const uint32_t* tileOrder, uint32_t tileFirst, uint32_t tileStride,
    uint32_t tileCount, uint32_t tilesX, uint32_t sppFirst, uint32_t frames, uint32_t passes, uint32_t ldsBytes, int collectStats, const uint32_t* blockDesc, uint32_t nBlocks, uint32_t* tileCost,
    uint32_t rankCount, unsigned long long* launchClk, hipStream_t stream);
uint32_t crt_render_resident_waves(int device, int kind, uint32_t ldsBytes);
hipError_t crt_launch_accumulate(const void* slab, void* acc, uint32_t tileFirst, uint32_t tileStride, uint32_t tileCount, uint32_t tilesX, uint32_t W, uint32_t frames, uint32_t passes,
    hipStream_t stream);
hipError_t crt_launch_find_nearest(const crt::Scene* sc, const void* rays, void* hits, uint32_t n, crt::Counters* counters, uint32_t ldsBytes, uint32_t* cursor, hipStream_t stream);
hipError_t crt_launch_is_occluded(const crt::Scene* sc, const void* rays, int32_t* occluded, uint32_t n, uint32_t ldsBytes, uint32_t* cursor, hipStream_t stream);
hipError_t crt_launch_whitted(const crt::Scene* sc, int accel, const crt::AltAccelDev* alt, const crt::TlasAltDev* tl, void* acc, uint32_t* pixels, crt::Counters* counters, uint32_t ldsBytes,
    hipStream_t stream);
size_t crt_whitted_inspect_work_bytes(uint32_t pixelCount);
hipError_t crt_launch_whitted_inspect(const crt::Scene* sc, int accel, const crt::AltAccelDev* alt, const crt::TlasAltDev* tl, int inspect, int32_t peakIn, void* acc, uint32_t* pixels,
    crt::Counters* counters, int32_t* trav, int32_t* tested, void* work, uint32_t ldsBytes, hipStream_t stream);
hipError_t crt_launch_resolve(const void* acc, uint32_t* pixels, float* tileSums, uint32_t tileFirst, uint32_t tileStride, uint32_t tileCount, uint32_t tilesX, uint32_t W, float scale,
    hipStream_t stream);
hipError_t crt_launch_commit_frame(const void* slabWindow, uint32_t frameInWindow, uint32_t passes, void* acc, uint32_t* pixels, float* tileSums, uint32_t tileFirst, uint32_t tileStride,
    uint32_t tileCount, uint32_t tilesX, uint32_t W, float scale, hipStream_t stream);

uint32_t crt_pool_streams(uint32_t frames);
size_t crt_pool_scratch_bytes_per_window(uint32_t tileCount);
hipError_t crt_launch_render_pool(const crt::Scene* sc, void* slab, void* facScratch, crt::Counters* counters, unsigned long long* tileClocks, const uint32_t* tileOrder, uint32_t tileFirst,
    uint32_t tileStride, uint32_t tileCount, uint32_t tilesX, uint32_t sppFirst, uint32_t frames, uint32_t passes, int collectStats, uint32_t rankFirst, uint32_t waveFrames,
    const uint32_t* waveTab, uint32_t tabBlocks, uint32_t longFrames, uint32_t* tileCost, unsigned long long* launchClk, hipStream_t stream);
uint32_t crt_pool_lds_bytes(uint32_t stackDepth, uint32_t streams);
int crt_debug_pool_stamps(unsigned long long* out, int reset);
int crt_debug_pool_density(unsigned long long* out, int reset);
size_t crt_debug_pool_timeline(unsigned long long* out, size_t cap);

uint32_t crt_probe_paths(void);
hipError_t crt_launch_probe(const crt::Scene* sc, uint32_t tileFirst, uint32_t tileStride, uint32_t tileCount, uint32_t tilesX, uint32_t* tileCost, hipStream_t stream);
hipError_t crt_launch_render_alt(int accel, const crt::Scene* sc, const crt::AltAccelDev* acc, const crt::TlasAltDev* tl, void* slab, crt::Counters* counters, uint32_t tileFirst, uint32_t tileStride,
    uint32_t tileCount, uint32_t tilesX, uint32_t sppFirst, uint32_t frames, uint32_t passes, hipStream_t stream);
hipError_t crt_launch_sample_query(int accel, const crt::Scene* sc, const crt::AltAccelDev* acc, const crt::TlasAltDev* tl, const void* rays, uint32_t* seeds, float* rgb, uint32_t n,
    crt::Counters* counters, uint32_t* cursor, uint32_t* residentLanes, hipStream_t stream);

hipError_t crt_launch_find_nearest_prim(const crt::PrimDev* p, const void* rays, void* hits, uint32_t n, hipStream_t stream);
hipError_t crt_launch_render_prim(const crt::Scene* sc, const crt::PrimDev* p, void* slab, crt::Counters* counters, uint32_t tileFirst, uint32_t tileStride, uint32_t tileCount, uint32_t tilesX,
    uint32_t sppFirst, uint32_t frames, uint32_t passes, hipStream_t stream);
hipError_t crt_launch_sample_query_prim(const crt::Scene* sc, const crt::PrimDev* p, const void* rays, uint32_t* seeds, float* rgb, uint32_t n, crt::Counters* counters, uint32_t* cursor,
    uint32_t* residentLanes, hipStream_t stream);
hipError_t crt_launch_probe_f64(int op, const void* in, void* out, uint32_t n, hipStream_t stream);

hipError_t crt_launch_find_nearest_alt(int kind, const crt::Scene* sc, const crt::AltAccelDev* acc, const void* rays, void* hits, uint32_t n, uint32_t* cursor, hipStream_t stream);
hipError_t crt_launch_is_occluded_alt(int kind, const crt::Scene* sc, const crt::AltAccelDev* acc, const void* rays, int32_t* occluded, uint32_t n, uint32_t* cursor, hipStream_t stream);
hipError_t crt_launch_tlas_alt_query(int kind, bool occl, const crt::Scene* sc, const crt::TlasAltDev* tl, const void* rays, void* out, uint32_t n, uint32_t* cursor, hipStream_t stream);

hipError_t crt_launch_hit_info(const crt::Scene* sc, const void* rays, const void* hits, void* out, uint32_t n, uint32_t objects, uint32_t fileTris, hipStream_t stream);
hipError_t crt_launch_sky_color(const crt::Scene* sc, const void* rays, float* rgb, uint32_t n, hipStream_t stream);
hipError_t crt_launch_refit(char* geom, uint32_t leafOff, uint32_t pairBase, uint32_t triBase, uint32_t triCount, const float* pos, const void* plan, const uint32_t* levelOff, uint32_t levels,
    uint32_t rootCode, float* out, hipStream_t stream);
hipError_t crt_launch_probe_f32(int op, const void* in, void* out, uint32_t n, hipStream_t stream);

uint32_t crt_grid_build_blocks(int device);
size_t crt_grid_scan_chunks(uint32_t cells);
hipError_t crt_launch_grid_bounds(const float* pos, uint32_t triCount, crt::GridBuildState* state, uint32_t maxBlocks, hipStream_t stream);
hipError_t crt_launch_grid_count(const float* pos, uint32_t triCount, const crt::GridParams* g, uint32_t cells, uint32_t* counts, unsigned long long* chunkSums, crt::GridBuildState* state,
    uint32_t maxBlocks, hipStream_t stream);
hipError_t crt_launch_grid_fill(const float* pos, uint32_t triCount, const crt::GridParams* g, uint32_t cells, const uint32_t* cellStart, uint32_t* cursor, int32_t* unsorted, int32_t* refs,
    uint32_t total, const char* geom, uint32_t leafOff, uint32_t triBase, int globalIdx, crt::AltTri* tris, uint32_t maxBlocks, hipStream_t stream);

hipError_t crt_launch_tlas_build(const char* geom, uint32_t instOff, const float* T, const float* rootBox, uint32_t blasCount, uint32_t pairRel, uint32_t instRel, void* out,
    hipStream_t stream);

uint32_t crt_debug_query_grid(void);

}

namespace crt {

inline uint32_t bounded_query_grid(uint32_t grid) { const uint32_t k = crt_debug_query_grid(); return (k != 0u && k < grid) ? k : grid; }

inline uint32_t query_grid(uint32_t n, uint32_t ldsBytes)
{
    uint32_t perCu = ldsBytes ? (160u * 1024u) / ldsBytes : 16u; if (perCu > 16u) perCu = 16u; if (perCu < 4u) perCu = 4u;
    const uint32_t need = (n + 63u) / 64u, fill = 256u * perCu;
    return bounded_query_grid(need < fill ? need : fill);
}

inline bool query_launch_begin(uint32_t n, uint32_t* cursor, hipStream_t stream, hipError_t* status)
{
    *status = hipSuccess;
    if (n == 0) return false;
    if (!cursor) { *status = hipErrorInvalidValue; return false; }
// ... 6 lines not shown
```

cpu-ray-tracer_amd/csrc/device/layout.h:

```cpp
#pragma once
#include <stdint.h>

namespace crt {

constexpr uint32_t kRefInterior = 0x80000000u;
constexpr uint32_t kRefTlasBit = 0x40000000u;
constexpr uint32_t kRefTlasInterior = 0x40000000u;
constexpr uint32_t kRefTlasLeaf = 0xC0000000u;
constexpr uint32_t kRefReturn = 0xFFFFFFFFu;
constexpr uint32_t kRefDone = 0u;
constexpr uint32_t kRefOffsetMask = 0x3fffffffu;
constexpr uint64_t kMaxGeomBytes = 1ull << 32;

constexpr uint32_t kRef16Interior = 0x8000u, kRef16TlasBit = 0x4000u, kRef16TlasLeaf = 0xC000u, kRef16TagMask = 0xC000u, kRef16IndexMask = 0x3fffu;
constexpr uint32_t kRef16Return = 0xFFFFu, kRef16MaxIndex = 0x3ffeu;

struct alignas(16) NodeChild { float lo[3]; uint32_t ref; float hi[3]; uint32_t ref16; };
struct alignas(64) NodePair { NodeChild c[2]; };

struct alignas(16) LeafTri {
    float v0[3]; uint32_t shadeIdx;
    float e1[3]; int32_t objIdx;
    float e2[3]; uint32_t remain;
};

struct alignas(16) ShadeTri {
    float n0[3], n1[3], n2[3];
    float uv0[2], uv1[2], uv2[2];
    int32_t mat;
};

struct alignas(16) TlasNode { float lo[3]; uint32_t ref; float hi[3]; uint32_t ref16; };

struct alignas(16) Instance {
    float invT[12];
    uint32_t shadeBase;
    uint32_t rootRef16;
    uint32_t rootRef;
    int32_t objIdx;
    float T[12];
    uint32_t triCount;
    uint32_t pad[3];
};

struct alignas(16) Material {
    float reflectivity, refractivity;
    float absorption[3];
    uint32_t texOffset;
    int32_t texW, texH;
};

struct Scene {
    int32_t kind;
    int32_t depthLimit;
    float camPos[3], topLeft[3], topRight[3], bottomLeft[3];
    float invW, invH;
    int32_t W, H;
    float lightInvT[12]; float lightNrm[3]; float lightSize;
    float lightPos[3];
    float floorN[3]; float floorD; float floorInvto;
    Material floorMat;
    uint32_t skyOffset; int32_t skyW, skyH;
    const char* geom;
    uint32_t tlasOff, instOff, shadeOff;
    uint32_t leafOff, tlasPairOff;
    uint32_t rootRef16, ref16ok;
    const uint32_t* texels;
    const Material* mats;
    uint32_t rootRef;
    uint32_t stackDepth;
    uint32_t bvhStack;
    uint32_t lightAxis, floorAxisY;
    uint32_t rootIsPair;
    float rootPair[16];
};

struct Counters { unsigned long long v[8]; };

struct alignas(16) RefitPlanRec { uint32_t pair, child[2], pad; };
constexpr uint32_t kPlanInterior = 0x80000000u;

struct alignas(64) TlasBuildHeader {
    uint32_t status;
    uint32_t step;
    uint32_t height;
    uint32_t searches;
    uint32_t staleA;
    uint32_t pad[11];
};
constexpr uint32_t kTlasBuildOk = 0u, kTlasBuildNoCandidate = 1u, kTlasBuildNoEnd = 2u;
constexpr uint32_t kTlasMaxBlas = 256u;

#if defined(__HIPCC__)
#define CRT_HOST_DEVICE __host__ __device__
#else
#define CRT_HOST_DEVICE
#endif
template <class TriCountOf>
CRT_HOST_DEVICE inline bool hit_record_ok(int32_t objIdx, int32_t triIdx, uint32_t objects, TriCountOf&& triCountOf)
{
    if (objIdx < 2) return objIdx >= -1;
    if ((uint32_t)(objIdx - 2) >= objects) return false;
    return triIdx >= 0 && (uint32_t)triIdx < triCountOf((uint32_t)(objIdx - 2));
}

struct KdNode { float lo[3]; int32_t left; float hi[3]; int32_t right; float splitDistance; int32_t splitAxis; uint32_t firstTri, triCount; };
struct AltTri { float v0[3]; uint32_t triIdx; float e1[3]; int32_t objIdx; float e2[3]; uint32_t pad; };
struct AltAccelDev {
    const KdNode* kdNodes; const uint32_t* kdRefs; uint32_t kdStack;
    const AltTri* tris;
    int32_t res[3]; float cell[3]; float lo[3], hi[3]; const uint32_t* cellStart; const int32_t* cellRefs;
};

struct BlasAltDesc {
    uint32_t nodeBase, refBase, triBase;
    uint32_t cellBase, cellRefBase;
    int32_t objIdx;
    int32_t res[3]; float cell[3]; float lo[3], hi[3];
};
struct TlasAltDev {
    const BlasAltDesc* desc;
    const void* kdNodes; const uint32_t* kdRefs; const void* tris;
    const uint32_t* cellStart; const int32_t* cellRefs;
    uint32_t kdStack;
};

struct GridParams { int32_t res[3]; float cell[3]; float lo[3]; };
struct alignas(16) GridBuildState { unsigned long long key[6]; unsigned long long total; uint32_t nonFinite; uint32_t pad; };

struct PrimDev {
    float quadInvT[12], quadNrm[3], quadSize;
    float spherePos[3], pad0;
    float cubeInvM[12], cubeM[12], cubeMin[3], cubeMax[3];
    float torusInvT[12], torusT[12], rt2, rc2, r2, pad1;
    float refl[11], refr[11], absorb[33];
    float pad2;
    const uint32_t* red; const uint32_t* blue;
};

}
```

cpu-ray-tracer_amd/csrc/device/probe.hip:

```cpp
#include "dev_common.h"
#include "launch.h"

namespace crt {

__global__ __launch_bounds__(256) void probe_f32_kernel(int op, const uint32_t* __restrict__ in, uint32_t* __restrict__ out, uint32_t n)
{
    const uint32_t i = blockIdx.x * 256u + threadIdx.x;
    if (i >= n) return;
    switch (op) {
    case 0: out[i] = asu(crt_expf(asf(in[i]))); break;
    case 1: out[i] = asu(crt_acosf(asf(in[i]))); break;
    case 2: out[i] = asu(crt_atan2f(asf(in[2 * (size_t)i]), asf(in[2 * (size_t)i + 1]))); break;
    case 3: out[i] = asu(__builtin_sqrtf(asf(in[i]))); break;
    case 4: out[i] = asu(asf(in[2 * (size_t)i]) / asf(in[2 * (size_t)i + 1])); break;
    case 5: {
        const uint32_t* p = in + 6 * (size_t)i; uint32_t* o = out + 7 * (size_t)i;
        const f3 a = mk3(asf(p[0]), asf(p[1]), asf(p[2])), b = mk3(asf(p[3]), asf(p[4]), asf(p[5]));
        const f3 nn = normalize3(a), cr = cross3(a, b);
        o[0] = asu(nn.x); o[1] = asu(nn.y); o[2] = asu(nn.z); o[3] = asu(cr.x); o[4] = asu(cr.y); o[5] = asu(cr.z); o[6] = asu(dot3(a, b));
        break;
    }
    case 6: {
        uint32_t* o = out + 18 * (size_t)i;
        uint32_t s = init_seed(in[i]);
        o[0] = s;
#pragma unroll
        for (int k = 0; k < 8; k++) o[1 + k] = asu(rnd(s));
#pragma unroll
        for (int k = 0; k < 8; k++) o[9 + k] = asu(rnd_pm1(s));
        o[17] = s;
        break;
    }
    case 7: {
        const uint32_t* p = in + 4 * (size_t)i;
        out[i] = tex_index(0u, (int)p[2], (int)p[3], asf(p[0]), asf(p[1]));
        break;
    }
    case 8: {
        const uint32_t* p = in + 5 * (size_t)i; uint32_t* o = out + 3 * (size_t)i;
        const f3 D = mk3(asf(p[0]), asf(p[1]), asf(p[2]));
        const float phi = crt_atan2f(-D.z, D.x) + CRT_PI;
        const float theta = crt_acosf(-D.y);
        o[0] = asu(phi); o[1] = asu(theta); o[2] = tex_index(0u, (int)p[3], (int)p[4], phi * CRT_INV2PI, theta * CRT_INVPI);
        break;
    }
    case 9: {
        const uint32_t* p = in + 13 * (size_t)i;
        rec4 lo, hi; lo.x = asf(p[0]); lo.y = asf(p[1]); lo.z = asf(p[2]); lo.w = 0.0f; hi.x = asf(p[3]); hi.y = asf(p[4]); hi.z = asf(p[5]); hi.w = 0.0f;
        const f3 O = mk3(asf(p[6]), asf(p[7]), asf(p[8])), rD = mk3(asf(p[9]), asf(p[10]), asf(p[11]));
        const float tray = asf(p[12]);
        out[2 * (size_t)i] = asu(box_exact(lo, hi, O, rD, tray)); out[2 * (size_t)i + 1] = asu(box_fast(lo, hi, O, rD, tray));
        break;
    }
    case 10: {
        const uint32_t* p = in + 16 * (size_t)i; uint32_t* o = out + 4 * (size_t)i;
        rec4 a, b, c;
        a.x = asf(p[0]); a.y = asf(p[1]); a.z = asf(p[2]); a.w = asf(7u);
        b.x = asf(p[3]); b.y = asf(p[4]); b.z = asf(p[5]); b.w = asf(2u);
        c.x = asf(p[6]); c.y = asf(p[7]); c.z = asf(p[8]); c.w = asf(1u);
        const f3 O = mk3(asf(p[9]), asf(p[10]), asf(p[11])), D = mk3(asf(p[12]), asf(p[13]), asf(p[14]));
        Hit h; h.t = asf(p[15]); h.u = 0.0f; h.v = 0.0f; h.objIdx = -1; h.triIdx = -1;
        hit_tri(a, b, c, O, D, h);
        o[0] = asu(h.t); o[1] = asu(h.u); o[2] = asu(h.v); o[3] = (h.triIdx == 7) ? 1u : 0u;
        break;
    }
    default: break;
    }
}

}

extern "C" hipError_t crt_launch_probe_f32(int op, const void* in, void* out, uint32_t n, hipStream_t stream)
{
    if (n == 0) return hipSuccess;
    if (op < 0 || op > 10) return hipErrorInvalidValue;
    hipLaunchKernelGGL(crt::probe_f32_kernel, dim3((n + 255u) / 256u), dim3(256), 0, stream, op, (const uint32_t*)in, (uint32_t*)out, n);
    return hipGetLastError();
}
```

cpu-ray-tracer_amd/csrc/device/render_pool.hip:

```cpp
#include "dev_common.h"
#include "launch.h"

namespace crt {

enum : uint32_t {
    F_OX = 0, F_OY, F_OZ, F_DX, F_DY, F_DZ,
    F_RX, F_RY, F_RZ,
    F_T,
    F_SEED, F_META,
    F_U, F_V,
    F_COUNT,
    F_CUR = F_U, F_PEND = F_V,
    F_TRI = F_RX
};
constexpr uint32_t kMetaItemMask = 0x7ffu, kMetaDepthShift = 11u, kMetaInside = 1u << 14, kMetaFresh = 1u << 15, kMetaObjShift = 16u, kMetaLowMask = 0xffffu;
constexpr uint32_t kQueueMask = 127u;

#ifndef CRT_POOL_MIN_WAVES
#define CRT_POOL_MIN_WAVES 4
#endif
#ifndef CRT_POOL_SHADE_MIN
#define CRT_POOL_SHADE_MIN 64
#endif
#ifndef CRT_POOL_NODE_STEPS
#define CRT_POOL_NODE_STEPS 2
#endif
#ifndef CRT_POOL_NODE2_MIN
#define CRT_POOL_NODE2_MIN 16
#endif
#ifndef CRT_POOL_STARVE
#define CRT_POOL_STARVE 40
#endif

#ifdef CRT_POOL_STAMPS
__device__ unsigned long long g_poolStamps[16];
#define CRT_PSTAMP(var) unsigned long long var; asm volatile("s_memtime %0\n\ts_waitcnt lgkmcnt(0)" : "=s"(var) :: "memory")
#define CRT_PACC(i, a, b) (pst[i] += (b) - (a))
#else
#define CRT_PSTAMP(var)
#define CRT_PACC(i, a, b)
#endif
#ifdef CRT_POOL_DENS
__device__ unsigned long long g_poolDens[48];
#define CRT_DENS(i, v) (dens[i] += (uint32_t)(v))
#define CRT_DENS_MASK(i, pred) (dens[i] += (uint32_t)__popcll(__builtin_amdgcn_ballot_w64(pred)))
#define CRT_LIVE_BUCKET(n) ((n) >= 112u ? 0u : (n) >= 96u ? 1u : (n) >= 64u ? 2u : 3u)
#else
#define CRT_DENS(i, v)
#define CRT_DENS_MASK(i, pred)
#endif
#ifdef CRT_POOL_TIMELINE
__device__ unsigned long long* g_poolTimeline = nullptr;
#endif
__device__ __forceinline__ bool lane_in(uint64_t m) { return __builtin_amdgcn_inverse_ballot_w64(m); }
__device__ __forceinline__ uint64_t finite3_mask(f3 v)
{
    const uint32_t m = 0x7f800000u;
    return __builtin_amdgcn_ballot_w64((asu(v.x) & m) != m) & __builtin_amdgcn_ballot_w64((asu(v.y) & m) != m) & __builtin_amdgcn_ballot_w64((asu(v.z) & m) != m);
}
__device__ __forceinline__ uint32_t rank_in(uint64_t m) { return __builtin_amdgcn_mbcnt_hi((uint32_t)(m >> 32), __builtin_amdgcn_mbcnt_lo((uint32_t)m, 0u)); }

template <int KIND, bool COUNT, int S>
__global__ __launch_bounds__(64, CRT_POOL_MIN_WAVES) void render_pool_kernel(const Scene sc, float4* __restrict__ slab, float* __restrict__ facScratch, Counters* __restrict__ counters,
                                                             unsigned long long* __restrict__ tileClocks, const uint32_t* __restrict__ tileOrder,
                                                             uint32_t tileFirst, uint32_t tileStride, uint32_t tileCount, uint32_t tilesX,
                                                             uint32_t sppFirst, uint32_t frames, uint32_t passes, uint32_t groups, uint32_t waveFrames, const uint32_t* __restrict__ waveTab, uint32_t tabBlocks, uint32_t longFrames,
                                                             uint32_t rankFirst, uint32_t* __restrict__ tileCost, unsigned long long* __restrict__ launchClk)
{
    extern __shared__ uint32_t lds[];
    const uint32_t lane = threadIdx.x;
#ifdef CRT_POOL_TIMELINE
    const unsigned long long tl0 = wall_clock64();
#endif
    const unsigned long long clk0 = (COUNT || tileCost) ? wall_clock64() : 0ull;
    if (launchClk && lane == 0) { atomicMax(&launchClk[0], ~clk0); atomicMax(&launchClk[1], clk0); }
    uint32_t rank0, grp, wf = waveFrames, first = 0u, limit = frames;
    if (waveTab) {
        if (blockIdx.x < tabBlocks) {
            uint32_t lo = 0u, hi = tileCount - rankFirst;
            while (hi - lo > 1u) { const uint32_t mid = (lo + hi) >> 1; if (waveTab[2u * mid] <= blockIdx.x) lo = mid; else hi = mid; }
            rank0 = lo; grp = blockIdx.x - waveTab[2u * lo]; wf = waveTab[2u * lo + 1u]; limit = longFrames;
        } else { const uint32_t b = blockIdx.x - tabBlocks; rank0 = b / groups; grp = b - rank0 * groups; wf = (uint32_t)S; first = longFrames; }
    } else { rank0 = blockIdx.x / groups; grp = blockIdx.x - rank0 * groups; }
    const uint32_t rank = rank0 + rankFirst;
    if (rank >= tileCount) return;
    const uint32_t tl = tileOrder ? tileOrder[rank] : rank;
    const uint32_t frame0 = first + grp * wf;
    if (frame0 >= limit) return;
    const uint32_t nOwn = (limit - frame0 < wf) ? limit - frame0 : wf;
    const uint32_t nStreams = nOwn < (uint32_t)S ? nOwn : (uint32_t)S;
    const uint32_t tile = tileFirst + tl * tileStride;
    const uint32_t tx = tile % tilesX, ty = tile / tilesX;
    const char* __restrict__ geom = sc.geom;
    float* __restrict__ fac = facScratch + (size_t)blockIdx.x * (15u * (uint32_t)S);

    char* const ldsB = reinterpret_cast<char*>(lds);
    const uint32_t laneB = lane * 2u;
    uint32_t* st = lds + (sc.stackDepth + 1u) * 32u;
    float* stf = reinterpret_cast<float*>(st);
    uint8_t* qEnd = reinterpret_cast<uint8_t*>(st + F_COUNT * S);
    uint8_t* qBnc = qEnd + 128, * qRdy = qEnd + 256;
    uint16_t* slotFrame = reinterpret_cast<uint16_t*>(qEnd + 384);
    auto stk_top = [&](uint32_t at) -> uint32_t { return *reinterpret_cast<const uint16_t*>(ldsB + at); };
    auto stk_put = [&](uint32_t at, uint32_t v) { *reinterpret_cast<uint16_t*>(ldsB + at) = (uint16_t)v; };

    Cnt cn; cn.rays = cn.primary = cn.interior = cn.leaf = cn.tri = cn.tlas = cn.visits = cn.meshhits = 0;
    uint32_t trips = 0;
#ifdef CRT_POOL_DENS
    uint32_t dens[48]; for (int i = 0; i < 48; i++) dens[i] = 0;
    uint32_t live = nStreams; unsigned long long liveClk = wall_clock64();
#endif
    const uint32_t items = 256u * passes;
    const uint32_t rowLen = 64u * passes;
    const f3 nil3 = mk3(0.0f, 0.0f, 0.0f);

    for (uint32_t s = lane; s < nStreams; s += 64u) {
        st[F_SEED * S + s] = init_seed(tx + ty * (uint32_t)sc.W + (sppFirst + (frame0 + s) * passes) * 1799u);
        st[F_META * S + s] = kMetaFresh;
        qEnd[s] = (uint8_t)s;
        if (S > 64) slotFrame[s] = (uint16_t)s;
    }
    uint32_t nextFrame = nStreams;
    uint32_t endH = 0, endT = nStreams, bncH = 0, bncT = 0, rdyH = 0, rdyT = 0;

    uint64_t mRes = 0ull;
    uint64_t mFinite = ~0ull;
    uint32_t sid = 0, cur = kRefDone, spB = laneB, metaLo = 0u;
    f3 tO = nil3, tD = nil3, trD = nil3;
    Hit h; h.t = 1e34f; h.u = 0; h.v = 0; h.objIdx = -1; h.triIdx = -1;
    rec4 q0 = {0, 0, 0, 0}, q1 = q0, q2 = q0, q3 = q0;

    auto new_ray = [&](bool act, uint32_t s, f3 v, bool norm, f3 O, uint32_t seed, uint32_t meta) {
        f3 D = v, rD = v; Hit nh; nh.t = 1e34f; nh.u = 0; nh.v = 0; nh.objIdx = -1; nh.triIdx = -1;
        uint32_t ncur = kRefDone, pend = 0u;
        if (act) {
            const float inv = rcp_exact(__builtin_sqrtf(dot3(v, v)));
            D = norm ? v * inv : v;
            rD = rcp_exact3(D);
            cn.rays++;
            {
                const kernarg_f lp = scene_floats(offsetof(Scene, lightInvT));
                const kernarg_f ax = scene_floats(offsetof(Scene, lightAxis));
                LightFloor lf;
#pragma unroll
                for (int i = 0; i < 12; i++) lf.lightInvT[i] = lp[i];
                lf.lightSize = lp[15]; lf.floorN[0] = lp[19]; lf.floorN[1] = lp[20]; lf.floorN[2] = lp[21]; lf.floorD = lp[22];
                lf.lightAxis = asu(ax[0]); lf.floorAxisY = asu(ax[1]);
                hit_light_floor(lf, O, D, nh);
            }
            if (sc.rootIsPair) {
                const kernarg_f rp = scene_floats(offsetof(Scene, rootPair));
                const rec4 a0 = {rp[0], rp[1], rp[2], rp[3]}, a1 = {rp[4], rp[5], rp[6], rp[7]};
                const rec4 b0 = {rp[8], rp[9], rp[10], rp[11]}, b1 = {rp[12], rp[13], rp[14], rp[15]};
                float d1, d2;
                if (__builtin_amdgcn_ballot_w64(!finite3(rD)) == 0ull) { d1 = box_fast(a0, a1, O, rD, nh.t); d2 = box_fast(b0, b1, O, rD, nh.t); }
                else { d1 = box_exact(a0, a1, O, rD, nh.t); d2 = box_exact(b0, b1, O, rD, nh.t); }
                const bool sw = d1 > d2;
                const float dn = sw ? d2 : d1, df = sw ? d1 : d2;
                const uint32_t rn = sw ? asu(b1.w) : asu(a1.w), rf = sw ? asu(a1.w) : asu(b1.w);
                const bool hitN = dn != 1e30f;
                pend = (hitN && df != 1e30f) ? rf : 0u;
                ncur = hitN ? rn : kRefDone;
                if (COUNT) { if (KIND == 0) cn.interior++; else cn.tlas++; }
            } else ncur = sc.rootRef16;
            if (COUNT && KIND == 0 && (ncur & kRef16TagMask) == 0u && ncur != kRefDone) cn.leaf++;
            stf[F_OX * S + s] = O.x; stf[F_OY * S + s] = O.y; stf[F_OZ * S + s] = O.z;
            stf[F_DX * S + s] = D.x; stf[F_DY * S + s] = D.y; stf[F_DZ * S + s] = D.z;
            stf[F_RX * S + s] = rD.x; stf[F_RY * S + s] = rD.y; stf[F_RZ * S + s] = rD.z;
            stf[F_T * S + s] = nh.t;
            st[F_SEED * S + s] = seed; st[F_META * S + s] = meta | ((uint32_t)(nh.objIdx + 1) << kMetaObjShift);
            st[F_CUR * S + s] = ncur; st[F_PEND * S + s] = pend;
        }
        const uint32_t depth = (meta >> kMetaDepthShift) & 7u;
        const uint64_t mAct = __builtin_amdgcn_ballot_w64(act);
        const uint64_t mW = mAct & __builtin_amdgcn_ballot_w64(ncur != kRefDone);
        const uint64_t mStop = __builtin_amdgcn_ballot_w64((uint32_t)(nh.objIdx + 1) <= 1u) | __builtin_amdgcn_ballot_w64((int)depth >= sc.depthLimit);
        const uint64_t mE = mAct & ~mW & mStop, mB = mAct & ~mW & ~mStop;
        CRT_DENS(20, __popcll(mAct)); CRT_DENS(19, __popcll(mW));
        if (lane_in(mW)) qRdy[(rdyT + rank_in(mW)) & kQueueMask] = (uint8_t)s;
        if (lane_in(mE)) qEnd[(endT + rank_in(mE)) & kQueueMask] = (uint8_t)s;
        if (lane_in(mB)) qBnc[(bncT + rank_in(mB)) & kQueueMask] = (uint8_t)s;
        rdyT += (uint32_t)__popcll(mW); endT += (uint32_t)__popcll(mE); bncT += (uint32_t)__popcll(mB);
    };
    auto world_ray = [&]() {
        tO = mk3(stf[F_OX * S + sid], stf[F_OY * S + sid], stf[F_OZ * S + sid]);
        tD = mk3(stf[F_DX * S + sid], stf[F_DY * S + sid], stf[F_DZ * S + sid]);
        trD = mk3(stf[F_RX * S + sid], stf[F_RY * S + sid], stf[F_RZ * S + sid]);
    };

    uint64_t mNode2 = 0ull;
    auto node_step = [&](uint64_t m) {
        const bool allFinite = (m & ~mFinite) == 0ull;
        if (lane_in(m)) {
            if (COUNT) { if (KIND == 1 && (cur & kRef16TlasBit) != 0u) cn.tlas++; else cn.interior++; }
            const uint32_t top = stk_top(spB);
            float d1, d2;
            if (__builtin_expect(allFinite, 1)) { d1 = box_fast(q0, q1, tO, trD, h.t); d2 = box_fast(q2, q3, tO, trD, h.t); }
            else { d1 = box_exact(q0, q1, tO, trD, h.t); d2 = box_exact(q2, q3, tO, trD, h.t); }
            const bool sw = d1 > d2;
            const float dn = sw ? d2 : d1, df = sw ? d1 : d2;
            const uint32_t rn = sw ? asu(q3.w) : asu(q1.w), rf = sw ? asu(q1.w) : asu(q3.w);
            stk_put(spB + 128u, rf);
            const bool hitN = dn != 1e30f, push = hitN && df != 1e30f;
            const bool pop = !hitN && spB != laneB;
            cur = hitN ? rn : (pop ? top : kRefDone);
            spB = spB + (push ? 128u : 0u) - (pop ? 128u : 0u);
            if (COUNT && (cur & kRef16TagMask) == 0u && cur != kRefDone) cn.leaf++;
        }
    };
    auto load_records = [&](uint64_t m) {
        const uint32_t idx = cur & kRef16IndexMask;
        const bool inter = (cur & kRef16Interior) != 0u;
        uint32_t oa = idx * (inter ? 64u : 48u) + (inter ? 0u : sc.leafOff - 48u);
        if (KIND == 1 && (cur & kRef16TlasBit) != 0u)
            oa = (cur & kRef16Interior) ? sc.instOff + idx * 128u : sc.tlasPairOff + idx * 64u;
        if (lane_in(m)) { q0 = ldg(geom, oa); q1 = ldg(geom, oa + 16u); q2 = ldg(geom, oa + 32u); q3 = ldg(geom, oa + 48u); }
    };

    auto tri_step = [&](uint64_t m) {
        CRT_DENS(3, 1); CRT_DENS(4, __popcll(m));
        if (lane_in(m)) {
            if (COUNT) cn.tri++;
            const uint32_t top = stk_top(spB);
            hit_tri(q0, q1, q2, tO, tD, h);
            const bool more = asu(q2.w) > 1u;
            const bool pop = !more && spB != laneB;
            const uint32_t next = more ? cur + 1u : (pop ? top : kRefDone);
            spB -= pop ? 128u : 0u;
            if (COUNT && !more && (next & kRef16TagMask) == 0u && next != kRefDone) cn.leaf++;
            cur = next;
        }
    };

#ifdef CRT_POOL_STAMPS
    unsigned long long pst[12] = {0, 0, 0, 0, 0, 0, 0, 0, 0, 0, 0, 0};
#endif
    for (;;) {
        CRT_PSTAMP(p0);
        if (mRes != 0ull) {
            uint64_t mNode, mTlas = 0ull;
            if (KIND == 0) mNode = mRes & __builtin_amdgcn_ballot_w64(cur > 0x7fffu);
            else { mTlas = mRes & __builtin_amdgcn_ballot_w64(cur >= kRef16TlasLeaf); mNode = mRes & __builtin_amdgcn_ballot_w64(cur - kRef16TlasBit < 0x8000u); }
            const uint64_t mTri = mRes & ~(mNode | mTlas);
            asm volatile("" : "+v"(q0), "+v"(q1), "+v"(q2), "+v"(q3));
            CRT_DENS(22, __popcll(mRes));
            if (mNode) { CRT_DENS(1, 1); CRT_DENS(2, __popcll(mNode)); }

            if (KIND == 1 && mTlas) { CRT_DENS(23, 1); CRT_DENS(24, __popcll(mTlas)); }
            uint64_t mBack = 0ull;
            if (KIND == 1 && mTlas != 0ull) {
                if (lane_in(mTlas)) {
                    if (COUNT) { cn.tlas++; cn.visits++; }
                    const f3 O = mk3(stf[F_OX * S + sid], stf[F_OY * S + sid], stf[F_OZ * S + sid]);
                    const f3 D = mk3(stf[F_DX * S + sid], stf[F_DY * S + sid], stf[F_DZ * S + sid]);
                    to_object_space(q0, q1, q2, O, D, tO, tD, trD);
                    spB += 128u; stk_put(spB, kRef16Return);
                    const uint32_t next = asu(q3.y);
                    if (COUNT && (next & kRef16TagMask) == 0u && next != kRefDone) cn.leaf++;
                    cur = next;
                }
                mFinite = (mFinite & ~mTlas) | (mTlas & finite3_mask(trD));
            }
            if (mNode != 0ull) node_step(mNode);
#if CRT_POOL_NODE_STEPS > 1
            uint64_t mLeafNow = 0ull;
#pragma unroll
            for (int rep = 1; rep < CRT_POOL_NODE_STEPS; rep++) {
                const uint64_t mStepped = rep == 1 ? mNode : mNode2;
                mNode2 = mStepped & (KIND == 0 ? __builtin_amdgcn_ballot_w64(cur > 0x7fffu) : __builtin_amdgcn_ballot_w64(cur - kRef16TlasBit < 0x8000u));
                if ((uint32_t)__popcll(mNode2) < (uint32_t)CRT_POOL_NODE2_MIN) { mNode2 = 0ull; break; }
                const uint64_t mLeaf = mStepped & __builtin_amdgcn_ballot_w64((cur & kRef16TagMask) == 0u) & ~__builtin_amdgcn_ballot_w64(cur == kRefDone);
                load_records(mNode2 | mLeaf);
                mLeafNow |= mLeaf;
                CRT_DENS(28, 1); CRT_DENS(29, __popcll(mNode2));
                node_step(mNode2);
            }
            const uint64_t mTriAll = mTri | mLeafNow;
            const uint64_t mTriRan = mTriAll;
#else
            const uint64_t mTriAll = mTri;
            const uint64_t mTriRan = mTriAll;
#endif
            if (mTriAll != 0ull) tri_step(mTriAll);
            if (KIND == 1) {
                mBack = (mNode | mTriRan) & __builtin_amdgcn_ballot_w64(cur == kRef16Return);
                if (mBack != 0ull) {
                    if (lane_in(mBack)) {
                        world_ray();
                        const bool pop = spB != laneB;
                        const uint32_t top = stk_top(spB);
                        cur = pop ? top : kRefDone; spB -= pop ? 128u : 0u;
                        if (COUNT && (cur & kRef16TagMask) == 0u && cur != kRefDone) cn.leaf++;
                    }
                    mFinite = (mFinite & ~mBack) | (mBack & finite3_mask(trD));
                }
            }
            asm volatile("" ::: "memory");
            const uint64_t mFin = mRes & __builtin_amdgcn_ballot_w64(cur == kRefDone);
            if (mFin != 0ull) {
                CRT_DENS(5, 1); CRT_DENS(6, __popcll(mFin));
                const uint32_t depth = (metaLo >> kMetaDepthShift) & 7u;
                const uint64_t mStop = __builtin_amdgcn_ballot_w64((uint32_t)(h.objIdx + 1) <= 1u) | __builtin_amdgcn_ballot_w64((int)depth >= sc.depthLimit);
                const uint64_t mE = mFin & mStop, mB = mFin & ~mStop;
                if (lane_in(mFin)) {
                    stf[F_T * S + sid] = h.t; stf[F_U * S + sid] = h.u; stf[F_V * S + sid] = h.v;
                    st[F_TRI * S + sid] = (uint32_t)h.triIdx;
                    st[F_META * S + sid] = metaLo | ((uint32_t)(h.objIdx + 1) << kMetaObjShift);
                }
                if (lane_in(mE)) qEnd[(endT + rank_in(mE)) & kQueueMask] = (uint8_t)sid;
                if (lane_in(mB)) qBnc[(bncT + rank_in(mB)) & kQueueMask] = (uint8_t)sid;
                endT += (uint32_t)__popcll(mE); bncT += (uint32_t)__popcll(mB);
                mRes &= ~mFin;
            }
            asm volatile("" ::: "memory");
        }
        CRT_PSTAMP(p1); CRT_PACC(0, p0, p1);
        if (__builtin_expect(mRes == 0ull, 0)) {
            if ((endT - endH) + (bncT - bncH) + (rdyT - rdyH) == 0u) break;
        }
        if (COUNT) trips++;
        CRT_DENS(0, 1);
#ifdef CRT_POOL_DENS
        dens[32u + CRT_LIVE_BUCKET(live)]++;
#endif
        {
            const uint32_t nRdy = rdyT - rdyH;
            const uint64_t mFree = ~mRes;
            if (nRdy != 0u) if (mFree != 0ull) {
                const uint32_t myRank = rank_in(mFree);
                const uint64_t mTake = mFree & __builtin_amdgcn_ballot_w64(myRank < nRdy);
                CRT_DENS(7, 1); CRT_DENS(8, __popcll(mTake));
                if (lane_in(mTake)) {
                    sid = qRdy[(rdyH + myRank) & kQueueMask];
                    tO = mk3(stf[F_OX * S + sid], stf[F_OY * S + sid], stf[F_OZ * S + sid]);
                    tD = mk3(stf[F_DX * S + sid], stf[F_DY * S + sid], stf[F_DZ * S + sid]);
                    trD = mk3(stf[F_RX * S + sid], stf[F_RY * S + sid], stf[F_RZ * S + sid]);
                    const uint32_t meta = st[F_META * S + sid];
                    h.t = stf[F_T * S + sid]; h.objIdx = (int)(meta >> kMetaObjShift) - 1; h.u = 0; h.v = 0; h.triIdx = -1;
                    metaLo = meta & kMetaLowMask;
                    cur = st[F_CUR * S + sid];
                    const uint32_t pend = st[F_PEND * S + sid];
                    stk_put(laneB + 128u, pend);
                    spB = laneB + (pend ? 128u : 0u);
                }
                mFinite = (mFinite & ~mTake) | (mTake & finite3_mask(trD));
                mRes |= mTake;
                rdyH += (uint32_t)__popcll(mTake);
            }
            if (mRes != 0ull) {
                CRT_DENS(21, 1);
                const uint32_t idx = cur & kRef16IndexMask;
                const bool inter = (cur & kRef16Interior) != 0u;
                uint32_t oa = idx * (inter ? 64u : 48u) + (inter ? 0u : sc.leafOff - 48u);
                if (KIND == 1 && (cur & kRef16TlasBit) != 0u)
                    oa = (cur & kRef16Interior) ? sc.instOff + idx * 128u : sc.tlasPairOff + idx * 64u;
                if (!lane_in(mRes)) oa = 0u;
                q0 = ldg(geom, oa); q1 = ldg(geom, oa + 16u); q2 = ldg(geom, oa + 32u); q3 = ldg(geom, oa + 48u);
            }
        }
        asm volatile("" ::: "memory");
        {
            const uint32_t nEnd = endT - endH, nBnc = bncT - bncH, nRdy = rdyT - rdyH, nRes = (uint32_t)__popcll(mRes);
            const bool starving = nRes + nRdy < (uint32_t)CRT_POOL_STARVE;
            bool runEnd = false, runBnc = false;
            if ((nEnd | nBnc) >= (uint32_t)CRT_POOL_SHADE_MIN || starving) {
                runEnd = nEnd >= (uint32_t)CRT_POOL_SHADE_MIN || (starving && nEnd > 0u && nEnd >= nBnc);
                runBnc = nBnc >= (uint32_t)CRT_POOL_SHADE_MIN || (starving && nBnc > nEnd);
            }

            CRT_PSTAMP(p2b); CRT_PACC(1, p1, p2b);
            if (runEnd) {
                const uint32_t n = nEnd < 64u ? nEnd : 64u;
                const bool act = lane < n;
                const uint32_t s = act ? qEnd[(endH + lane) & kQueueMask] : 0u;
                endH += n;
                uint32_t meta = 0, seed = 0; int obj = -1; f3 D = nil3;
                if (act) { meta = st[F_META * S + s]; seed = st[F_SEED * S + s]; obj = (int)(meta >> kMetaObjShift) - 1; D = mk3(stf[F_DX * S + s], stf[F_DY * S + s], stf[F_DZ * S + s]); }
                const bool first = (meta & kMetaFresh) != 0u;
                const int depth = (int)((meta >> kMetaDepthShift) & 7u);
                uint32_t item = meta & kMetaItemMask;
                const bool ended = act && !first, miss = ended && obj == -1;
#ifdef CRT_POOL_DENS
                dens[36u + CRT_LIVE_BUCKET(live)]++;
#endif
                CRT_DENS(9, 1); CRT_DENS(10, n); CRT_DENS_MASK(11, miss); CRT_DENS_MASK(13, act && first); CRT_DENS_MASK(25, ended && depth > 0); CRT_DENS_MASK(26, ended && depth > 1); CRT_DENS_MASK(27, ended && depth > 2);
                if (ended && obj >= 2) cn.meshhits++;
                float fk[15];
#pragma unroll
                for (int k = 0; k < 5; k++) {
                    fk[3 * k] = fk[3 * k + 1] = fk[3 * k + 2] = 0.0f;
                    if (ended && depth > k) {
#pragma unroll
                        for (int j = 0; j < 3; j++) fk[3 * k + j] = __hip_atomic_load(fac + (3 * k + j) * S + s, __ATOMIC_RELAXED, __HIP_MEMORY_SCOPE_AGENT);
                    }
                }
                uint32_t skyTexel = 0u;
                if (miss) {
                    const float phi = crt_atan2f(-D.z, D.x) + CRT_PI, theta = crt_acosf(-D.y);
                    const kernarg_f sk = scene_floats(offsetof(Scene, skyOffset));
                    skyTexel = sc.texels[tex_index(asu(sk[0]), (int)asu(sk[1]), (int)asu(sk[2]), phi * CRT_INV2PI, theta * CRT_INVPI)];
                }
                bool gen = act && first;
                size_t sampleAt = 0;
                if (ended) {
                    uint32_t pix = item, pass = 0;
                    if (passes != 1u) { pix = item / passes; pass = item - pix * passes; }
                    const uint32_t fr = frame0 + (S > 64 ? (uint32_t)slotFrame[s] : s);
                    sampleAt = (((size_t)(fr >> 6) * tileCount + tl) * 256u + pix) * rowLen + ((fr & 63u) * passes + pass);
                    item++;
                    gen = item < items;
                }
                if (S > 64) if (nextFrame < nOwn) {
                    const uint64_t mDone = __builtin_amdgcn_ballot_w64(ended) & ~__builtin_amdgcn_ballot_w64(gen);
                    if (mDone != 0ull) {
                        const uint32_t f = nextFrame + rank_in(mDone);
                        const uint64_t mTake = mDone & __builtin_amdgcn_ballot_w64(f < nOwn);
                        if (lane_in(mTake)) {
                            slotFrame[s] = (uint16_t)f;
                            seed = init_seed(tx + ty * (uint32_t)sc.W + (sppFirst + (frame0 + f) * passes) * 1799u);
                            item = 0u; gen = true;
                        }
                        nextFrame += (uint32_t)__popcll(mTake);
                    }
                }
#ifdef CRT_POOL_DENS
                {
                    const uint32_t gone = (uint32_t)__popcll(__builtin_amdgcn_ballot_w64(ended) & ~__builtin_amdgcn_ballot_w64(gen));
                    if (gone) { const unsigned long long now = wall_clock64(); dens[44u + CRT_LIVE_BUCKET(live)] += (uint32_t)(now - liveClk); liveClk = now; live -= gone; }
                }
#endif
                const kernarg_f cam = scene_floats(offsetof(Scene, camPos));
                const f3 camPos = mk3(cam[0], cam[1], cam[2]);
                f3 v = camPos;
                if (gen) {
                    const uint32_t pix = (passes == 1u) ? item : item / passes;
                    const int x = (int)(tx * 16u + (pix & 15u)), y = (int)(ty * 16u + (pix >> 4));
                    const float jy = rnd(seed);
                    const float jx = rnd(seed);
                    const float u = ((float)x + jx) * cam[12], vv = ((float)y + jy) * cam[13];
                    const f3 TL = mk3(cam[3], cam[4], cam[5]), TR = mk3(cam[6], cam[7], cam[8]), BL = mk3(cam[9], cam[10], cam[11]);
                    const f3 P = TL + u * (TR - TL) + vv * (BL - TL);
                    v = P - camPos;
                    cn.primary++;
                }
                CRT_DENS_MASK(12, gen);
                CRT_PSTAMP(e1); CRT_PACC(2, p2b, e1);
                new_ray(gen, s, v, true, camPos, seed, item);
                CRT_PSTAMP(e2); CRT_PACC(3, e1, e2);
                if (ended) {
                    f3 L = miss ? tex_unpack(skyTexel) : ((depth >= sc.depthLimit) ? mk3(0, 0, 0) : mk3(24, 24, 22));
#pragma unroll
                    for (int k = 4; k >= 0; k--)
                        if (depth > k) L = mk3(fk[3 * k], fk[3 * k + 1], fk[3 * k + 2]) * L;
                    slab[sampleAt] = make_float4(L.x, L.y, L.z, 0.0f);
                }
#ifdef CRT_POOL_STAMPS
                { CRT_PSTAMP(e3); CRT_PACC(4, e2, e3); pst[10]++; }
#endif
                asm volatile("" :: "v"(fk[0]), "v"(fk[1]), "v"(fk[2]), "v"(fk[3]), "v"(fk[4]), "v"(fk[5]), "v"(fk[6]), "v"(fk[7]), "v"(fk[8]), "v"(fk[9]), "v"(fk[10]), "v"(fk[11]), "v"(fk[12]), "v"(fk[13]), "v"(fk[14]), "v"(skyTexel));
            }
            CRT_PSTAMP(p3);
            asm volatile("" ::: "memory");
            if (runBnc) {
                const uint32_t n = nBnc < 64u ? nBnc : 64u;
                const bool act = lane < n;
                const uint32_t s = act ? qBnc[(bncH + lane) & kQueueMask] : 0u;
                bncH += n;
                f3 O = nil3, D = nil3; float ht = 0, hu = 0, hv = 0; int obj = 1; uint32_t tri = 0, seed = 0, meta = 0;
                if (act) {
                    tri = st[F_TRI * S + s];
                    O = mk3(stf[F_OX * S + s], stf[F_OY * S + s], stf[F_OZ * S + s]);
                    D = mk3(stf[F_DX * S + s], stf[F_DY * S + s], stf[F_DZ * S + s]);
                    ht = stf[F_T * S + s]; hu = stf[F_U * S + s]; hv = stf[F_V * S + s];
                    seed = st[F_SEED * S + s]; meta = st[F_META * S + s]; obj = (int)(meta >> kMetaObjShift) - 1;
                }
                const bool mesh = act && obj >= 2;
#ifdef CRT_POOL_DENS
                dens[40u + CRT_LIVE_BUCKET(live)]++;
#endif
                CRT_DENS(14, 1); CRT_DENS(15, n); CRT_DENS_MASK(16, mesh);
                rec4 s0 = {0, 0, 0, 0}, s1 = s0, s2 = s0, s3 = s0;
                if (mesh) { const uint32_t so = sc.shadeOff + tri * 64u; s0 = ldg(geom, so); s1 = ldg(geom, so + 16u); s2 = ldg(geom, so + 32u); s3 = ldg(geom, so + 48u); cn.meshhits++; }
                const bool inside = (meta & kMetaInside) != 0u;
                const int depth = (int)((meta >> kMetaDepthShift) & 7u);
                const uint32_t item = meta & kMetaItemMask;
                float tu = 0, tv = 0; uint32_t tOff = 0; int tW = 0, tH = 0;
                f3 I = O, N = O, absorb = O; float refl = 0, refr = 0;
                f3 v = O, pre = O; bool norm = false, diffuse = false, newInside = false;
                if (act) {
                    I = O + ht * D;
                    if (obj == 1) {
                        const kernarg_f fl = scene_floats(offsetof(Scene, floorN));
                        const kernarg_f fm = scene_floats(offsetof(Scene, floorMat));
                        N = mk3(fl[0], fl[1], fl[2]);
                        if (N.y == 1) {
                            float u = I.x, vv = I.z;
                            u *= fl[4]; vv *= fl[4];
                            tu = u - __builtin_floorf(u); tv = vv - __builtin_floorf(vv);
                        }
                        refl = fm[0]; refr = fm[1];
                        absorb = mk3(fm[2], fm[3], fm[4]);
                        tOff = asu(fm[5]); tW = (int)asu(fm[6]); tH = (int)asu(fm[7]);
                    } else {
                        const f3 n0 = mk3(s0.x, s0.y, s0.z), n1 = mk3(s0.w, s1.x, s1.y), n2 = mk3(s1.z, s1.w, s2.x);
                        const float w = 1 - hu - hv;
                        const f3 Nn = w * n0 + hu * n1 + hv * n2;
                        tu = w * s2.y + hu * s2.w + hv * s3.y;
                        tv = w * s2.z + hu * s3.x + hv * s3.z;
                        const rec4* mp = reinterpret_cast<const rec4*>(sc.mats + (int)asu(s3.w));
                        const rec4 m0 = mp[0], m1 = mp[1];
                        refl = m0.x; refr = m0.y; absorb = mk3(m0.z, m0.w, m1.x);
                        tOff = asu(m1.y); tW = (int)asu(m1.z); tH = (int)asu(m1.w);
                        if (KIND == 0) {
                            N = normalize3(Nn);
                        } else {
                            const uint32_t io = sc.instOff + (uint32_t)(obj - 2) * 128u + 64u;
                            const rec4 r0 = ldg(geom, io), r1 = ldg(geom, io + 16), r2 = ldg(geom, io + 32);
                            N = normalize3(mk3(r0.x * Nn.x + r0.y * Nn.y + r0.z * Nn.z + r0.w * 0.0f,
                                               r1.x * Nn.x + r1.y * Nn.y + r1.z * Nn.z + r1.w * 0.0f,
                                               r2.x * Nn.x + r2.y * Nn.y + r2.z * Nn.z + r2.w * 0.0f));
                        }
                    }
                    if (dot3(N, D) > 0) N = -N;
                    uint32_t texel = 0x00ffffffu;
                    if (tW > 0) texel = sc.texels[tex_index(tOff, tW, tH, tu, tv)];
                    f3 medium = mk3(1, 1, 1);
                    if (inside) {
                        const f3 ab = absorb * -ht;
                        medium = mk3(crt_expf(ab.x), crt_expf(ab.y), crt_expf(ab.z));
                    }
                    CRT_PSTAMP(b1); CRT_PACC(5, p3, b1);
                    const float r = rnd(seed);
                    const bool mirror = r < refl, dielectric = !mirror && r < refl + refr;
                    if (mirror) {
                        v = D - 2.0f * N * dot3(N, D);
                    } else if (dielectric) {
                        v = D - 2.0f * N * dot3(N, D);
                        const float n1 = inside ? 1.2f : 1, n2 = inside ? 1 : 1.2f;
                        const float eta = n1 / n2, cosi = dot3(-D, N);
                        const float cost2 = 1.0f - eta * eta * (1 - cosi * cosi);
                        if (cost2 > 0) {
                            const float a = n1 - n2, b2 = n1 + n2, R0 = (a * a) / (b2 * b2), cc = 1 - cosi;
                            const float Fr = R0 + (1 - R0) * (cc * cc * cc * cc * cc);
                            const f3 T = eta * D + ((eta * cosi - __builtin_sqrtf(__builtin_fabsf(cost2))) * N);
                            if (rnd(seed) > Fr) { v = T; newInside = !inside; }
                        }
                    } else {
                        f3 Rr;
                        do {
                            const float rz = rnd_pm1(seed);
                            const float ry = rnd_pm1(seed);
                            const float rx = rnd_pm1(seed);
                            Rr = mk3(rx, ry, rz);
                        } while (dot3(Rr, Rr) > 1);
                        if (dot3(Rr, N) < 0) Rr = Rr * -1.0f;
                        v = Rr; norm = true; diffuse = true;
                    }
                    const f3 c = (tW > 0) ? tex_unpack(texel) : mk3(1.0f, 1.0f, 1.0f);
                    if (diffuse) {
                        const f3 brdf = c * CRT_INVPI;
                        pre = medium * brdf * 2.0f * CRT_PI;
                    } else pre = c * medium;
                    CRT_PSTAMP(b2); CRT_PACC(6, b1, b2);
                    const float inv = rcp_exact(__builtin_sqrtf(dot3(v, v)));
                    const f3 nv = norm ? v * inv : v;
                    v = nv;
                    const f3 factor = diffuse ? pre * dot3(nv, N) : pre;
                    float* fd = fac + (3 * depth) * S + s;
                    __hip_atomic_store(fd, factor.x, __ATOMIC_RELAXED, __HIP_MEMORY_SCOPE_AGENT);
                    __hip_atomic_store(fd + S, factor.y, __ATOMIC_RELAXED, __HIP_MEMORY_SCOPE_AGENT);
                    __hip_atomic_store(fd + 2 * S, factor.z, __ATOMIC_RELAXED, __HIP_MEMORY_SCOPE_AGENT);
                    O = I + nv * CRT_EPS;
                    CRT_PSTAMP(b3); CRT_PACC(7, b2, b3);
                }
                CRT_PSTAMP(b4);
                new_ray(act, s, v, false, O, seed, item | ((uint32_t)(depth + 1) << kMetaDepthShift) | (newInside ? kMetaInside : 0u));
#ifdef CRT_POOL_STAMPS
                { CRT_PSTAMP(b5); CRT_PACC(8, b4, b5); pst[11]++; }
#endif
                asm volatile("" :: "v"(s0), "v"(s1), "v"(s2), "v"(s3));
            }
#ifdef CRT_POOL_STAMPS
            pst[9]++;
#endif
        }
    }
#ifdef CRT_POOL_STAMPS
    if (lane == 0) for (int i = 0; i < 12; i++) atomicAdd(&g_poolStamps[i], pst[i]);
#endif
#ifdef CRT_POOL_DENS
    dens[44u + CRT_LIVE_BUCKET(live)] += (uint32_t)(wall_clock64() - liveClk);
    if (lane == 0) for (int i = 0; i < 48; i++) if (dens[i]) atomicAdd(&g_poolDens[i], (unsigned long long)dens[i]);
#endif

#ifdef CRT_POOL_TIMELINE
    if (lane == 0 && g_poolTimeline) { uint32_t hw; asm volatile("s_getreg_b32 %0, hwreg(HW_REG_HW_ID)" : "=s"(hw)); g_poolTimeline[3 * (size_t)blockIdx.x] = tl0; g_poolTimeline[3 * (size_t)blockIdx.x + 1] = wall_clock64(); g_poolTimeline[3 * (size_t)blockIdx.x + 2] = hw; }
#endif
    if (tileCost && lane == 0 && nOwn == (uint32_t)S) atomicMax(&tileCost[tl], (uint32_t)((wall_clock64() - clk0) * 64ull / (uint32_t)S));
    if (launchClk && lane == 0) { const unsigned long long now = wall_clock64(), last = __hip_atomic_load(&launchClk[1], __ATOMIC_RELAXED, __HIP_MEMORY_SCOPE_AGENT), from = last > clk0 ? last : clk0; if (now > from) atomicAdd(&launchClk[2], now - from); }
    if (COUNT && tileClocks && lane == 0 && nOwn == frames) {
        tileClocks[2 * tl] = wall_clock64() - clk0;
        tileClocks[2 * tl + 1] = trips;
    }
    uint32_t vals[8] = {cn.rays, cn.primary, cn.interior, cn.leaf, cn.tri, cn.tlas, cn.visits, cn.meshhits};
#pragma unroll
    for (int i = 0; i < 8; i++) {
        if (!COUNT && i >= 2 && i != 7) continue;
        uint32_t sum = wave_sum(vals[i]);
        if (lane == 0 && sum) atomicAdd(&counters->v[i], (unsigned long long)sum);
    }
}

}

#ifndef CRT_POOL_STREAMS
#define CRT_POOL_STREAMS 128
#endif
extern "C" uint32_t crt_pool_streams(uint32_t frames) { return frames > 64u ? (uint32_t)CRT_POOL_STREAMS : 64u; }
#ifndef CRT_POOL_EXTRA_LDS
#define CRT_POOL_EXTRA_LDS 0
#endif
extern "C" uint32_t crt_pool_lds_bytes(uint32_t stackDepth, uint32_t streams) { return (stackDepth + 1u) * 64u * 2u + crt::F_COUNT * streams * 4u + 3u * 128u + (streams > 64u ? 2u * streams : 0u) + (uint32_t)CRT_POOL_EXTRA_LDS; }
extern "C" size_t crt_pool_scratch_bytes_per_window(uint32_t tileCount) { return (size_t)tileCount * 128u * 15u * 4u; }

#ifdef CRT_POOL_STAMPS
extern "C" int crt_debug_pool_stamps(unsigned long long* out, int reset)
{
    if (out && hipMemcpyFromSymbol(out, HIP_SYMBOL(crt::g_poolStamps), 128) != hipSuccess) return -1;
    if (reset) { unsigned long long z[16] = {}; if (hipMemcpyToSymbol(HIP_SYMBOL(crt::g_poolStamps), z, 128) != hipSuccess) return -1; }
    return 0;
}
#endif
#ifdef CRT_POOL_DENS
extern "C" int crt_debug_pool_density(unsigned long long* out, int reset)
{
    if (out && hipMemcpyFromSymbol(out, HIP_SYMBOL(crt::g_poolDens), 384) != hipSuccess) return -1;
    if (reset) { unsigned long long z[48] = {}; if (hipMemcpyToSymbol(HIP_SYMBOL(crt::g_poolDens), z, 384) != hipSuccess) return -1; }
    return 0;
}
#endif
#ifdef CRT_POOL_TIMELINE
static unsigned long long* g_timelineHost = nullptr; static size_t g_timelineCount = 0;
extern "C" size_t crt_debug_pool_timeline(unsigned long long* out, size_t cap)
{
    const size_t n = g_timelineCount < cap ? g_timelineCount : cap;
    if (out && n) (void)hipMemcpy(out, g_timelineHost, n * 24, hipMemcpyDeviceToHost);
    return g_timelineCount;
}
#endif
extern "C" hipError_t crt_launch_render_pool(const crt::Scene* sc, void* slab, void* facScratch, crt::Counters* counters, unsigned long long* tileClocks, const uint32_t* tileOrder,
                                             uint32_t tileFirst, uint32_t tileStride, uint32_t tileCount, uint32_t tilesX, uint32_t sppFirst,
                                             uint32_t frames, uint32_t passes, int collectStats, uint32_t rankFirst, uint32_t waveFrames, const uint32_t* waveTab, uint32_t tabBlocks, uint32_t longFrames,
                                             uint32_t* tileCost, unsigned long long* launchClk, hipStream_t stream)
{
    if (tileCount == 0 || frames == 0) return hipSuccess;
    if (!sc->ref16ok) return hipErrorInvalidValue;
    const uint32_t S = crt_pool_streams(frames);
    const uint32_t wf = (S == 64u || waveFrames < S) ? S : waveFrames;
    if (wf % S != 0u || wf > 0xff80u) return hipErrorInvalidValue;
// ... 21 lines not shown
```

Before: 30290 Mrays/s.

## Precompute camera-relative primary data, custom exact sqrt, fast sky angles, load offset hints

Result: faster. 30650 Mrays/s, median of 6 (+1.2%).

```diff
diff --git a/cpu-ray-tracer_amd/csrc/abi.cpp b/cpu-ray-tracer_amd/csrc/abi.cpp
--- a/cpu-ray-tracer_amd/csrc/abi.cpp
+++ b/cpu-ray-tracer_amd/csrc/abi.cpp
@@ -327,6 +327,7 @@
     s.bottomLeft[0] = -aspect; s.bottomLeft[1] = -1; s.bottomLeft[2] = 0;
     s.W = cfg->width; s.H = cfg->height; s.invW = 1.0f / cfg->width; s.invH = 1.0f / cfg->height;
     s.depthLimit = c->cfg.depthLimit;
+    crt::set_primary(s);
     if ((e = hipStreamSynchronize(c->stream)) != hipSuccess) return bail(e, "hipStreamSynchronize");
     *out = c;
     return CRT_OK;
@@ -620,6 +621,7 @@
         s.rootIsPair = 1;
     }
     if (hook("CRT_DEBUG_NO_ROOTPAIR")) s.rootIsPair = 0;
+    crt::set_primary(s);
     s.stackDepth = s.bvhStack + ((sd->kind == CRT_SCENE_TLAS) ? tlasHeight + 1 : 0);
     c->ldsBytes = s.stackDepth * 64u * 4u; c->latSlots = 0;
     if (const char* e = hook("CRT_DEBUG_EXTRA_LDS")) c->ldsBytes += (uint32_t)atoi(e);
@@ -746,6 +748,7 @@
         s.rootIsPair = 1;
     }
     if (hook("CRT_DEBUG_NO_ROOTPAIR")) s.rootIsPair = 0;
+    crt::set_primary(s);
     memcpy(c->meshLo, lo, 12); memcpy(c->meshHi, hi, 12); c->orderDirty = true;
 }
 
@@ -861,6 +864,7 @@
     crt::Scene& s = c->hScene;
     if (!memcmp(s.camPos, camPos, 12) && !memcmp(s.topLeft, tl, 12) && !memcmp(s.topRight, tr, 12) && !memcmp(s.bottomLeft, bl, 12)) return CRT_OK;
     memcpy(s.camPos, camPos, 12); memcpy(s.topLeft, tl, 12); memcpy(s.topRight, tr, 12); memcpy(s.bottomLeft, bl, 12);
+    crt::set_primary(s);
     c->orderDirty = true; c->epoch++;
     return CRT_OK;
 }
@@ -2712,23 +2716,65 @@
     return CRT_OK;
 }
 
-extern "C" int crt_debug_device_probe(crt_ctx* c, int op, const void* in, void* out, uint32_t n)
-{
-    static const uint8_t words[17][2] = {{1, 1}, {1, 1}, {2, 1}, {1, 1}, {2, 1}, {6, 7}, {1, 18}, {4, 1}, {5, 3}, {13, 2}, {16, 4}, {2, 2}, {2, 2}, {2, 2}, {2, 2}, {4, 2}, {2, 1}};
-    if (!c || !in || !out || op < 0 || op > 16 || n > (1u << 25)) return CRT_ERR_INVALID;
+extern "C" int crt_debug_check_sqrt(crt_ctx* c, uint64_t* out)
+{
+    if (!c || !out) return CRT_ERR_INVALID;
+    HIPCK(c, hipSetDevice(c->cfg.device));
+    unsigned long long* d = nullptr;
+    HIPCK(c, hipMalloc(&d, 16));
+    hipError_t e = hipMemsetAsync(d, 0, 16, c->stream);
+    if (e == hipSuccess) e = crt_launch_check_sqrt(d, c->stream);
+    if (e == hipSuccess) e = hipMemcpyAsync(out, d, 16, hipMemcpyDeviceToHost, c->stream);
+    if (e == hipSuccess) e = hipStreamSynchronize(c->stream);
+    (void)hipFree(d);
+    HIPCK(c, e);
+    return CRT_OK;
+}
+
+extern "C" int crt_debug_primary_block(crt_ctx* c, float* out, float* camera, float* lightFloor)
+{
+    if (!c || !out) return CRT_ERR_INVALID;
+    const crt::Scene& s = c->hScene;
+    static_assert(offsetof(crt::Scene, primRoot) == offsetof(crt::Scene, rootPair) + 64 && offsetof(crt::Scene, primDown) + 12 == offsetof(crt::Scene, rootPair) + 64 + 4 * crt::kPrimFloats, "primary block");
+    memcpy(out, s.rootPair, 64 + 4 * crt::kPrimFloats);
+    if (camera) memcpy(camera, s.camPos, 48);
+    if (lightFloor) { lightFloor[0] = s.lightInvT[7]; lightFloor[1] = s.lightInvT[3]; lightFloor[2] = s.lightInvT[11]; lightFloor[3] = s.floorD; }
+    return CRT_OK;
+}
+extern "C" int crt_debug_primary_block_host(int op, const float* in, float* out)
+{
+    static crt::Scene s{};
+    if (!in || !out || op < 0 || op > 2) return CRT_ERR_INVALID;
+    if (op == 0) {
+        s = crt::Scene{};
+        s.camPos[2] = -2; s.topLeft[0] = -1; s.topLeft[1] = 1; s.topRight[0] = 1; s.topRight[1] = 1; s.bottomLeft[0] = -1; s.bottomLeft[1] = -1;
+        memcpy(s.lightInvT, in, 48); s.floorD = in[12]; memcpy(s.rootPair, in + 13, 64); s.rootIsPair = 1;
+    } else if (op == 1) { memcpy(s.camPos, in, 12); memcpy(s.topLeft, in + 3, 12); memcpy(s.topRight, in + 6, 12); memcpy(s.bottomLeft, in + 9, 12); }
+    else memcpy(s.rootPair, in, 64);
+    crt::set_primary(s);
+    memcpy(out, s.rootPair, 64 + 4 * crt::kPrimFloats);
+    return CRT_OK;
+}
+
+static int device_probe(crt_ctx* c, int op, const void* in, void* out, uint32_t n)
+{
+    static const uint8_t words[18][2] = {{1, 1}, {1, 1}, {2, 1}, {1, 1}, {2, 1}, {6, 7}, {1, 18}, {4, 1}, {5, 3}, {13, 2}, {16, 4}, {2, 2}, {2, 2}, {2, 2}, {2, 2}, {4, 2}, {2, 1}, {5, 3}};
+    if (!c || !in || !out || op < 0 || op > 17 || n > (1u << 25)) return CRT_ERR_INVALID;
     if (n == 0) return CRT_OK;
     const size_t inBytes = (size_t)n * words[op][0] * 4, outBytes = (size_t)n * words[op][1] * 4;
     HIPCK(c, hipSetDevice(c->cfg.device));
     char* d = nullptr;
     HIPCK(c, hipMalloc((void**)&d, inBytes + outBytes));
     hipError_t e = hipMemcpyAsync(d, in, inBytes, hipMemcpyHostToDevice, c->stream);
-    if (e == hipSuccess) e = (op <= 10) ? crt_launch_probe_f32(op, d, d + inBytes, n, c->stream) : crt_launch_probe_f64(op, d, d + inBytes, n, c->stream);
+    if (e == hipSuccess) e = (op <= 10 || op == 17) ? crt_launch_probe_f32(op, d, d + inBytes, n, c->stream) : crt_launch_probe_f64(op, d, d + inBytes, n, c->stream);
     if (e == hipSuccess) e = hipMemcpyAsync(out, d + inBytes, outBytes, hipMemcpyDeviceToHost, c->stream);
     if (e == hipSuccess) e = hipStreamSynchronize(c->stream);
     (void)hipFree(d);
     HIPCK(c, e);
     return CRT_OK;
 }
+extern "C" int crt_debug_device_probe(crt_ctx* c, int op, const void* in, void* out, uint32_t n) { return (op > 16) ? CRT_ERR_INVALID : device_probe(c, op, in, out, n); }
+extern "C" int crt_debug_sky_probe(crt_ctx* c, const void* in, void* out, uint32_t n) { return device_probe(c, 17, in, out, n); }
 
 extern "C" int crt_debug_plan_job(const uint32_t* cost, uint32_t n, uint32_t windows, uint32_t frames, int pool, double poolWindowTicks,
                                   uint32_t* table, uint32_t tableCap, uint32_t* head, uint32_t* order)
diff --git a/cpu-ray-tracer_amd/csrc/device/dev_common.h b/cpu-ray-tracer_amd/csrc/device/dev_common.h
--- a/cpu-ray-tracer_amd/csrc/device/dev_common.h
+++ b/cpu-ray-tracer_amd/csrc/device/dev_common.h
@@ -42,7 +42,21 @@
     if (__builtin_expect(__builtin_amdgcn_ballot_w64(!okay) != 0, 0)) r = mk3(1.0f / v.x, 1.0f / v.y, 1.0f / v.z);
     return r;
 }
-__device__ __forceinline__ f3 normalize3(f3 v) { float inv = rcp_exact(__builtin_sqrtf(dot3(v, v))); return v * inv; }
+__device__ __forceinline__ float sqrt_exact(float x)
+{
+#ifdef CRT_DIET_NO_SQRT
+    return __builtin_sqrtf(x);
+#else
+    const float s = __builtin_amdgcn_sqrtf(x);
+    const float dn = __uint_as_float(__float_as_uint(s) - 1u), up = __uint_as_float(__float_as_uint(s) + 1u);
+    const float rdn = __builtin_fmaf(-dn, s, x), rup = __builtin_fmaf(-up, s, x);
+    float r = (rdn <= 0.0f) ? dn : s;
+    r = (rup > 0.0f) ? up : r;
+    if (__builtin_expect(__builtin_amdgcn_ballot_w64(__float_as_uint(x) - 0x0f800000u >= 0x70000000u) != 0, 0)) r = __builtin_sqrtf(x);
+    return r;
+#endif
+}
+__device__ __forceinline__ f3 normalize3(f3 v) { float inv = rcp_exact(sqrt_exact(dot3(v, v))); return v * inv; }
 __device__ __forceinline__ float min_std(float a, float b) { return (b < a) ? b : a; }
 __device__ __forceinline__ float max_std(float a, float b) { return (a < b) ? b : a; }
 __device__ __forceinline__ float min_tm(float a, float b) { return a < b ? a : b; }
@@ -121,12 +135,37 @@
 __device__ __forceinline__ float crt_acosf(float x)
 {
     const bool hi = x > 0.5f, lo = x < -0.5f;
-    const float s = __builtin_sqrtf(0.5f * (1.0f - __builtin_fabsf(x)));
+    const float s = sqrt_exact(0.5f * (1.0f - __builtin_fabsf(x)));
     const float p = crt_asin_small((hi || lo) ? s : x);
     float r = hi ? 2.0f * p : (lo ? CRT_PI - 2.0f * p : 1.5707963267948966f - p);
     if (x > 1.0f || x < -1.0f) r = asf(0x7fc00000u);
     return (x != x) ? x : r;
 }
+__device__ __forceinline__ float crt_atan2f_plain(float y, float x)
+{
+    const uint32_t sy = asu(y) & 0x80000000u, sx = asu(x) & 0x80000000u;
+    const float ax = __builtin_fabsf(x), ay = __builtin_fabsf(y);
+    const float a = crt_atan_pos(ay / ax);
+    const float r = sx ? (CRT_PI - a) : a;
+    return asf(asu(r) | sy);
+}
+__device__ __forceinline__ float crt_acosf_plain(float x)
+{
+    const bool hi = x > 0.5f, lo = x < -0.5f;
+    const float s = sqrt_exact(0.5f * (1.0f - __builtin_fabsf(x)));
+    const float p = crt_asin_small((hi || lo) ? s : x);
+    return hi ? 2.0f * p : (lo ? CRT_PI - 2.0f * p : 1.5707963267948966f - p);
+}
+__device__ __forceinline__ void sky_angles(f3 D, float& phi, float& theta)
+{
+    const float y = -D.z, x = D.x, c = -D.y;
+#ifndef CRT_DIET_NO_SKY
+    const uint64_t special = __builtin_amdgcn_uicmp((asu(x) << 1) - 1u, 0xfeffffffu, 35 ) | __builtin_amdgcn_uicmp((asu(y) << 1) - 1u, 0xfeffffffu, 35)
+                           | __builtin_amdgcn_ballot_w64(!(__builtin_fabsf(c) <= 1.0f));
+    if (__builtin_expect(special == 0, 1)) { phi = crt_atan2f_plain(y, x) + CRT_PI; theta = crt_acosf_plain(c); return; }
+#endif
+    phi = crt_atan2f(y, x) + CRT_PI; theta = crt_acosf(c);
+}
 
 __device__ __forceinline__ uint32_t wang_hash(uint32_t s)
 {
@@ -151,34 +190,50 @@
 typedef float rec4 __attribute__((ext_vector_type(4)));
 __device__ __forceinline__ rec4 ld4(const void* p) { return *reinterpret_cast<const rec4*>(p); }
 __device__ __forceinline__ rec4 ldg(const char* __restrict__ base, uint32_t byteOff) { return *reinterpret_cast<const rec4*>(base + byteOff); }
+static_assert(kMaxGeomBytes == (1ull << 32), "ldp: byteOff + 63 < 2^32");
+template <uint32_t PIECE> __device__ __forceinline__ rec4 ldp(const char* __restrict__ base, uint32_t byteOff)
+{
+#ifndef CRT_DIET_NO_RECPTR
+    __builtin_assume(byteOff <= 0xffffffffu - 63u);
+#endif
+    return ldg(base, byteOff + 16u * PIECE);
+}
 __device__ __forceinline__ bool finite3(f3 v)
 {
     const uint32_t m = 0x7f800000u;
     return ((asu(v.x) & m) != m) && ((asu(v.y) & m) != m) && ((asu(v.z) & m) != m);
 }
 
-__device__ __forceinline__ float box_exact(rec4 lo, rec4 hi, f3 O, f3 rD, float tray)
-{
-    float tx1 = (lo.x - O.x) * rD.x, tx2 = (hi.x - O.x) * rD.x;
+__device__ __forceinline__ float box_exact_rel(f3 lo, f3 hi, f3 rD, float tray)
+{
+    float tx1 = lo.x * rD.x, tx2 = hi.x * rD.x;
     float tmin = min_std(tx1, tx2), tmax = max_std(tx1, tx2);
-    float ty1 = (lo.y - O.y) * rD.y, ty2 = (hi.y - O.y) * rD.y;
+    float ty1 = lo.y * rD.y, ty2 = hi.y * rD.y;
     tmin = max_std(tmin, min_std(ty1, ty2)); tmax = min_std(tmax, max_std(ty1, ty2));
-    float tz1 = (lo.z - O.z) * rD.z, tz2 = (hi.z - O.z) * rD.z;
+    float tz1 = lo.z * rD.z, tz2 = hi.z * rD.z;
     tmin = max_std(tmin, min_std(tz1, tz2)); tmax = min_std(tmax, max_std(tz1, tz2));
     return (tmax >= tmin && tmin < tray && tmax > 0) ? tmin : 1e30f;
+}
+__device__ __forceinline__ float box_exact(rec4 lo, rec4 hi, f3 O, f3 rD, float tray)
+{
+    return box_exact_rel(mk3(lo.x - O.x, lo.y - O.y, lo.z - O.z), mk3(hi.x - O.x, hi.y - O.y, hi.z - O.z), rD, tray);
 }
 __device__ __forceinline__ float vmin(float a, float b) { float r; asm("v_min_f32 %0, %1, %2" : "=v"(r) : "v"(a), "v"(b)); return r; }
 __device__ __forceinline__ float vmax(float a, float b) { float r; asm("v_max_f32 %0, %1, %2" : "=v"(r) : "v"(a), "v"(b)); return r; }
 __device__ __forceinline__ float vmin3(float a, float b, float c) { float r; asm("v_min3_f32 %0, %1, %2, %3" : "=v"(r) : "v"(a), "v"(b), "v"(c)); return r; }
 __device__ __forceinline__ float vmax3(float a, float b, float c) { float r; asm("v_max3_f32 %0, %1, %2, %3" : "=v"(r) : "v"(a), "v"(b), "v"(c)); return r; }
-__device__ __forceinline__ float box_fast(rec4 lo, rec4 hi, f3 O, f3 rD, float tray)
-{
-    float tx1 = (lo.x - O.x) * rD.x, tx2 = (hi.x - O.x) * rD.x;
-    float ty1 = (lo.y - O.y) * rD.y, ty2 = (hi.y - O.y) * rD.y;
-    float tz1 = (lo.z - O.z) * rD.z, tz2 = (hi.z - O.z) * rD.z;
+__device__ __forceinline__ float box_fast_rel(f3 lo, f3 hi, f3 rD, float tray)
+{
+    float tx1 = lo.x * rD.x, tx2 = hi.x * rD.x;
+    float ty1 = lo.y * rD.y, ty2 = hi.y * rD.y;
+    float tz1 = lo.z * rD.z, tz2 = hi.z * rD.z;
     float tmin = vmax3(vmin(tx1, tx2), vmin(ty1, ty2), vmin(tz1, tz2));
     float tmax = vmin3(vmax(tx1, tx2), vmax(ty1, ty2), vmax(tz1, tz2));
     return (tmax >= tmin && tmin < tray && tmax > 0) ? tmin : 1e30f;
+}
+__device__ __forceinline__ float box_fast(rec4 lo, rec4 hi, f3 O, f3 rD, float tray)
+{
+    return box_fast_rel(mk3(lo.x - O.x, lo.y - O.y, lo.z - O.z), mk3(hi.x - O.x, hi.y - O.y, hi.z - O.z), rD, tray);
 }
 
 __device__ __forceinline__ void hit_tri(rec4 a, rec4 b, rec4 c, f3 O, f3 D, Hit& h)
@@ -196,18 +251,19 @@
     if (ok) { h.t = t; h.u = u; h.v = v; h.triIdx = (int)asu(a.w); h.objIdx = (int)asu(b.w); }
 }
 
-struct LightFloor { float lightInvT[12]; float lightSize; uint32_t lightAxis, floorAxisY; float floorN[3]; float floorD; };
+struct LightFloor { float lightInvT[12]; float lightSize; uint32_t lightAxis, floorAxisY; float floorN[3]; float floorD; float preOy, preOx, preOz, preNum; };
+template <bool PRE = false>
 __device__ __forceinline__ void hit_light_floor(const LightFloor& sc, f3 O, f3 D, Hit& h)
 {
     {
         const float* c = sc.lightInvT;
         float Oy, Dy;
-        if (sc.lightAxis) { Oy = O.y + c[7]; Dy = D.y; }
+        if (sc.lightAxis) { Oy = PRE ? sc.preOy : O.y + c[7]; Dy = D.y; }
         else { Oy = c[4] * O.x + c[5] * O.y + c[6] * O.z + c[7]; Dy = c[4] * D.x + c[5] * D.y + c[6] * D.z; }
         const float t = Oy / -Dy;
         if (t < h.t && t > 0) {
             float Ox, Oz, Dx, Dz;
-            if (sc.lightAxis) { Ox = O.x + c[3]; Oz = O.z + c[11]; Dx = D.x; Dz = D.z; }
+            if (sc.lightAxis) { Ox = PRE ? sc.preOx : O.x + c[3]; Oz = PRE ? sc.preOz : O.z + c[11]; Dx = D.x; Dz = D.z; }
             else {
                 Ox = c[0] * O.x + c[1] * O.y + c[2] * O.z + c[3];
                 Oz = c[8] * O.x + c[9] * O.y + c[10] * O.z + c[11];
@@ -221,7 +277,7 @@
     }
     {
         float num, den;
-        if (sc.floorAxisY) { num = O.y + sc.floorD; den = D.y; }
+        if (sc.floorAxisY) { num = PRE ? sc.preNum : O.y + sc.floorD; den = D.y; }
         else { const f3 N = mk3(sc.floorN[0], sc.floorN[1], sc.floorN[2]); num = dot3(O, N) + sc.floorD; den = dot3(D, N); }
         const float t = -num / den;
         if (t < h.t && t > 0) { h.t = t; h.objIdx = 1; }
@@ -235,6 +291,7 @@
     for (int i = 0; i < 12; i++) lf.lightInvT[i] = sc.lightInvT[i];
     lf.lightSize = sc.lightSize; lf.lightAxis = sc.lightAxis; lf.floorAxisY = sc.floorAxisY;
     lf.floorN[0] = sc.floorN[0]; lf.floorN[1] = sc.floorN[1]; lf.floorN[2] = sc.floorN[2]; lf.floorD = sc.floorD;
+    lf.preOy = lf.preOx = lf.preOz = lf.preNum = 0.0f;
     hit_light_floor(lf, O, D, h);
 }
 
@@ -257,6 +314,7 @@
 static_assert(offsetof(Scene, topLeft) == offsetof(Scene, camPos) + 12 && offsetof(Scene, bottomLeft) == offsetof(Scene, camPos) + 36 && offsetof(Scene, invW) == offsetof(Scene, camPos) + 48 && offsetof(Scene, invH) == offsetof(Scene, camPos) + 52, "camera block");
 static_assert(offsetof(Scene, lightSize) == offsetof(Scene, lightInvT) + 60 && offsetof(Scene, floorN) == offsetof(Scene, lightInvT) + 76 && offsetof(Scene, floorD) == offsetof(Scene, lightInvT) + 88 && offsetof(Scene, floorInvto) == offsetof(Scene, floorN) + 16, "light / floor block");
 static_assert(offsetof(Scene, floorAxisY) == offsetof(Scene, lightAxis) + 4 && offsetof(Scene, skyW) == offsetof(Scene, skyOffset) + 4 && offsetof(Scene, skyH) == offsetof(Scene, skyOffset) + 8, "flag / sky words");
+static_assert(offsetof(Scene, primRoot) == offsetof(Scene, rootPair) + 64 && offsetof(Scene, primFloor) == offsetof(Scene, primLight) + 12 && offsetof(Scene, primDown) == offsetof(Scene, primRight) + 12, "camera-relative block");
 static_assert(offsetof(Material, absorption) == 8 && offsetof(Material, texOffset) == 20 && offsetof(Material, texW) == 24 && offsetof(Material, texH) == 28, "Material words");
 typedef const float __attribute__((address_space(4)))* kernarg_f;
 __device__ __forceinline__ kernarg_f scene_floats(size_t byteOffset)
@@ -371,8 +429,8 @@
 
 __device__ __forceinline__ f3 sky_color(const Scene& sc, f3 D)
 {
-    float phi = crt_atan2f(-D.z, D.x) + CRT_PI;
-    float theta = crt_acosf(-D.y);
+    float phi, theta;
+    sky_angles(D, phi, theta);
     return tex_sample(sc, sc.skyOffset, sc.skyW, sc.skyH, phi * CRT_INV2PI, theta * CRT_INVPI);
 }
 
diff --git a/cpu-ray-tracer_amd/csrc/device/kernels.hip b/cpu-ray-tracer_amd/csrc/device/kernels.hip
--- a/cpu-ray-tracer_amd/csrc/device/kernels.hip
+++ b/cpu-ray-tracer_amd/csrc/device/kernels.hip
@@ -1045,6 +1045,25 @@
     return hipGetLastError();
 }
 
+namespace crt {
+__global__ __launch_bounds__(256) void check_sqrt_kernel(unsigned long long* out)
+{
+    const uint32_t tid = blockIdx.x * 256u + threadIdx.x, nthreads = gridDim.x * 256u;
+    unsigned long long n = 0, bad = 0;
+    for (uint64_t b = tid; b < (1ull << 32); b += nthreads) {
+        const float x = asf((uint32_t)b);
+        n++;
+        if (!same_bits(sqrt_exact(x), __builtin_sqrtf(x))) bad++;
+    }
+    atomicAdd(&out[0], n); atomicAdd(&out[1], bad);
+}
+}
+extern "C" hipError_t crt_launch_check_sqrt(unsigned long long* out, hipStream_t stream)
+{
+    hipLaunchKernelGGL(crt::check_sqrt_kernel, dim3(4096), dim3(256), 0, stream, out);
+    return hipGetLastError();
+}
+
 extern "C" hipError_t crt_launch_render(const crt::Scene* sc, void* slab, crt::Counters* counters, unsigned long long* tileClocks, const uint32_t* tileOrder,
                                         uint32_t tileFirst, uint32_t tileStride, uint32_t tileCount, uint32_t tilesX, uint32_t sppFirst,
                                         uint32_t frames, uint32_t passes, uint32_t ldsBytes, int collectStats, const uint32_t* blockDesc, uint32_t nBlocks, uint32_t* tileCost, uint32_t rankCount, unsigned long long* launchClk, hipStream_t stream)
diff --git a/cpu-ray-tracer_amd/csrc/device/launch.h b/cpu-ray-tracer_amd/csrc/device/launch.h
--- a/cpu-ray-tracer_amd/csrc/device/launch.h
+++ b/cpu-ray-tracer_amd/csrc/device/launch.h
@@ -6,6 +6,7 @@
 extern "C" {
 
 hipError_t crt_launch_check_reciprocals(unsigned long long* out, hipStream_t stream);
+hipError_t crt_launch_check_sqrt(unsigned long long* out, hipStream_t stream);
 hipError_t crt_launch_render(const crt::Scene* sc, void* slab, crt::Counters* counters, unsigned long long* tileClocks, const uint32_t* tileOrder, uint32_t tileFirst, uint32_t tileStride,
     uint32_t tileCount, uint32_t tilesX, uint32_t sppFirst, uint32_t frames, uint32_t passes, uint32_t ldsBytes, int collectStats, const uint32_t* blockDesc, uint32_t nBlocks, uint32_t* tileCost,
     uint32_t rankCount, unsigned long long* launchClk, hipStream_t stream);
diff --git a/cpu-ray-tracer_amd/csrc/device/layout.h b/cpu-ray-tracer_amd/csrc/device/layout.h
--- a/cpu-ray-tracer_amd/csrc/device/layout.h
+++ b/cpu-ray-tracer_amd/csrc/device/layout.h
@@ -73,7 +73,25 @@
     uint32_t lightAxis, floorAxisY;
     uint32_t rootIsPair;
     float rootPair[16];
+    float primRoot[12];
+    float primLight[3];
+    float primFloor;
+    float primRight[3], primDown[3];
 };
+constexpr uint32_t kPrimFloats = 22u;
+
+inline void set_primary(Scene& s)
+{
+    const float* O = s.camPos;
+    for (int c = 0; c < 2; c++)
+        for (int k = 0; k < 3; k++) {
+            s.primRoot[6 * c + k] = s.rootPair[8 * c + k] - O[k];
+            s.primRoot[6 * c + 3 + k] = s.rootPair[8 * c + 4 + k] - O[k];
+        }
+    s.primLight[0] = O[1] + s.lightInvT[7]; s.primLight[1] = O[0] + s.lightInvT[3]; s.primLight[2] = O[2] + s.lightInvT[11];
+    s.primFloor = O[1] + s.floorD;
+    for (int k = 0; k < 3; k++) { s.primRight[k] = s.topRight[k] - s.topLeft[k]; s.primDown[k] = s.bottomLeft[k] - s.topLeft[k]; }
+}
 
 struct Counters { unsigned long long v[8]; };
 
diff --git a/cpu-ray-tracer_amd/csrc/device/probe.hip b/cpu-ray-tracer_amd/csrc/device/probe.hip
--- a/cpu-ray-tracer_amd/csrc/device/probe.hip
+++ b/cpu-ray-tracer_amd/csrc/device/probe.hip
@@ -44,6 +44,13 @@
         o[0] = asu(phi); o[1] = asu(theta); o[2] = tex_index(0u, (int)p[3], (int)p[4], phi * CRT_INV2PI, theta * CRT_INVPI);
         break;
     }
+    case 17: {
+        const uint32_t* p = in + 5 * (size_t)i; uint32_t* o = out + 3 * (size_t)i;
+        float phi, theta;
+        sky_angles(mk3(asf(p[0]), asf(p[1]), asf(p[2])), phi, theta);
+        o[0] = asu(phi); o[1] = asu(theta); o[2] = tex_index(0u, (int)p[3], (int)p[4], phi * CRT_INV2PI, theta * CRT_INVPI);
+        break;
+    }
     case 9: {
         const uint32_t* p = in + 13 * (size_t)i;
         rec4 lo, hi; lo.x = asf(p[0]); lo.y = asf(p[1]); lo.z = asf(p[2]); lo.w = 0.0f; hi.x = asf(p[3]); hi.y = asf(p[4]); hi.z = asf(p[5]); hi.w = 0.0f;
@@ -73,7 +80,7 @@
 extern "C" hipError_t crt_launch_probe_f32(int op, const void* in, void* out, uint32_t n, hipStream_t stream)
 {
     if (n == 0) return hipSuccess;
-    if (op < 0 || op > 10) return hipErrorInvalidValue;
+    if ((op < 0 || op > 10) && op != 17) return hipErrorInvalidValue;
     hipLaunchKernelGGL(crt::probe_f32_kernel, dim3((n + 255u) / 256u), dim3(256), 0, stream, op, (const uint32_t*)in, (uint32_t*)out, n);
     return hipGetLastError();
 }
diff --git a/cpu-ray-tracer_amd/csrc/device/render_pool.hip b/cpu-ray-tracer_amd/csrc/device/render_pool.hip
--- a/cpu-ray-tracer_amd/csrc/device/render_pool.hip
+++ b/cpu-ray-tracer_amd/csrc/device/render_pool.hip
@@ -1,3 +1,4 @@
+#include <type_traits>
 #include "dev_common.h"
 #include "launch.h"
 
@@ -55,8 +56,13 @@
 __device__ __forceinline__ bool lane_in(uint64_t m) { return __builtin_amdgcn_inverse_ballot_w64(m); }
 __device__ __forceinline__ uint64_t finite3_mask(f3 v)
 {
+#ifdef CRT_DIET_NO_MASKS
     const uint32_t m = 0x7f800000u;
     return __builtin_amdgcn_ballot_w64((asu(v.x) & m) != m) & __builtin_amdgcn_ballot_w64((asu(v.y) & m) != m) & __builtin_amdgcn_ballot_w64((asu(v.z) & m) != m);
+#else
+    const float inf = __builtin_inff();
+    return __builtin_amdgcn_fcmpf(__builtin_fabsf(v.x), inf, 4) & __builtin_amdgcn_fcmpf(__builtin_fabsf(v.y), inf, 4) & __builtin_amdgcn_fcmpf(__builtin_fabsf(v.z), inf, 4);
+#endif
 }
 __device__ __forceinline__ uint32_t rank_in(uint64_t m) { return __builtin_amdgcn_mbcnt_hi((uint32_t)(m >> 32), __builtin_amdgcn_mbcnt_lo((uint32_t)m, 0u)); }
 
@@ -130,11 +136,16 @@
     Hit h; h.t = 1e34f; h.u = 0; h.v = 0; h.objIdx = -1; h.triIdx = -1;
     rec4 q0 = {0, 0, 0, 0}, q1 = q0, q2 = q0, q3 = q0;
 
-    auto new_ray = [&](bool act, uint32_t s, f3 v, bool norm, f3 O, uint32_t seed, uint32_t meta) {
+    auto new_ray = [&](auto primary, bool act, uint32_t s, f3 v, bool norm, f3 O, uint32_t seed, uint32_t meta) {
+#ifdef CRT_DIET_NO_CAMREL
+        constexpr bool PRIM = false;
+#else
+        constexpr bool PRIM = decltype(primary)::value;
+#endif
         f3 D = v, rD = v; Hit nh; nh.t = 1e34f; nh.u = 0; nh.v = 0; nh.objIdx = -1; nh.triIdx = -1;
         uint32_t ncur = kRefDone, pend = 0u;
         if (act) {
-            const float inv = rcp_exact(__builtin_sqrtf(dot3(v, v)));
+            const float inv = rcp_exact(sqrt_exact(dot3(v, v)));
             D = norm ? v * inv : v;
             rD = rcp_exact3(D);
             cn.rays++;
@@ -146,14 +157,24 @@
                 for (int i = 0; i < 12; i++) lf.lightInvT[i] = lp[i];
                 lf.lightSize = lp[15]; lf.floorN[0] = lp[19]; lf.floorN[1] = lp[20]; lf.floorN[2] = lp[21]; lf.floorD = lp[22];
                 lf.lightAxis = asu(ax[0]); lf.floorAxisY = asu(ax[1]);
-                hit_light_floor(lf, O, D, nh);
+                lf.preOy = lf.preOx = lf.preOz = lf.preNum = 0.0f;
+                if constexpr (PRIM) {
+                    constexpr size_t pl = (offsetof(Scene, primLight) - offsetof(Scene, lightInvT)) / 4;
+                    lf.preOy = lp[pl]; lf.preOx = lp[pl + 1]; lf.preOz = lp[pl + 2]; lf.preNum = lp[pl + 3];
+                }
+                hit_light_floor<PRIM>(lf, O, D, nh);
             }
             if (sc.rootIsPair) {
                 const kernarg_f rp = scene_floats(offsetof(Scene, rootPair));
                 const rec4 a0 = {rp[0], rp[1], rp[2], rp[3]}, a1 = {rp[4], rp[5], rp[6], rp[7]};
                 const rec4 b0 = {rp[8], rp[9], rp[10], rp[11]}, b1 = {rp[12], rp[13], rp[14], rp[15]};
                 float d1, d2;
-                if (__builtin_amdgcn_ballot_w64(!finite3(rD)) == 0ull) { d1 = box_fast(a0, a1, O, rD, nh.t); d2 = box_fast(b0, b1, O, rD, nh.t); }
+                const bool allFinite = (__builtin_amdgcn_ballot_w64(true) & ~finite3_mask(rD)) == 0ull;
+                if constexpr (PRIM) {
+                    const f3 ra0 = mk3(rp[16], rp[17], rp[18]), ra1 = mk3(rp[19], rp[20], rp[21]), rb0 = mk3(rp[22], rp[23], rp[24]), rb1 = mk3(rp[25], rp[26], rp[27]);
+                    if (allFinite) { d1 = box_fast_rel(ra0, ra1, rD, nh.t); d2 = box_fast_rel(rb0, rb1, rD, nh.t); }
+                    else { d1 = box_exact_rel(ra0, ra1, rD, nh.t); d2 = box_exact_rel(rb0, rb1, rD, nh.t); }
+                } else if (allFinite) { d1 = box_fast(a0, a1, O, rD, nh.t); d2 = box_fast(b0, b1, O, rD, nh.t); }
                 else { d1 = box_exact(a0, a1, O, rD, nh.t); d2 = box_exact(b0, b1, O, rD, nh.t); }
                 const bool sw = d1 > d2;
                 const float dn = sw ? d2 : d1, df = sw ? d1 : d2;
@@ -214,7 +235,7 @@
         uint32_t oa = idx * (inter ? 64u : 48u) + (inter ? 0u : sc.leafOff - 48u);
         if (KIND == 1 && (cur & kRef16TlasBit) != 0u)
             oa = (cur & kRef16Interior) ? sc.instOff + idx * 128u : sc.tlasPairOff + idx * 64u;
-        if (lane_in(m)) { q0 = ldg(geom, oa); q1 = ldg(geom, oa + 16u); q2 = ldg(geom, oa + 32u); q3 = ldg(geom, oa + 48u); }
+        if (lane_in(m)) { q0 = ldp<0>(geom, oa); q1 = ldp<1>(geom, oa); q2 = ldp<2>(geom, oa); q3 = ldp<3>(geom, oa); }
     };
 
     auto tri_step = [&](uint64_t m) {
@@ -355,7 +376,7 @@
                 if (KIND == 1 && (cur & kRef16TlasBit) != 0u)
                     oa = (cur & kRef16Interior) ? sc.instOff + idx * 128u : sc.tlasPairOff + idx * 64u;
                 if (!lane_in(mRes)) oa = 0u;
-                q0 = ldg(geom, oa); q1 = ldg(geom, oa + 16u); q2 = ldg(geom, oa + 32u); q3 = ldg(geom, oa + 48u);
+                q0 = ldp<0>(geom, oa); q1 = ldp<1>(geom, oa); q2 = ldp<2>(geom, oa); q3 = ldp<3>(geom, oa);
             }
         }
         asm volatile("" ::: "memory");
@@ -396,7 +417,7 @@
                 }
                 uint32_t skyTexel = 0u;
                 if (miss) {
-                    const float phi = crt_atan2f(-D.z, D.x) + CRT_PI, theta = crt_acosf(-D.y);
+                    float phi, theta; sky_angles(D, phi, theta);
                     const kernarg_f sk = scene_floats(offsetof(Scene, skyOffset));
                     skyTexel = sc.texels[tex_index(asu(sk[0]), (int)asu(sk[1]), (int)asu(sk[2]), phi * CRT_INV2PI, theta * CRT_INVPI)];
                 }
@@ -438,14 +459,21 @@
                     const float jy = rnd(seed);
                     const float jx = rnd(seed);
                     const float u = ((float)x + jx) * cam[12], vv = ((float)y + jy) * cam[13];
-                    const f3 TL = mk3(cam[3], cam[4], cam[5]), TR = mk3(cam[6], cam[7], cam[8]), BL = mk3(cam[9], cam[10], cam[11]);
-                    const f3 P = TL + u * (TR - TL) + vv * (BL - TL);
+                    const f3 TL = mk3(cam[3], cam[4], cam[5]);
+#ifdef CRT_DIET_NO_CAMREL
+                    const f3 TR = mk3(cam[6], cam[7], cam[8]), BL = mk3(cam[9], cam[10], cam[11]);
+                    const f3 right = TR - TL, down = BL - TL;
+#else
+                    constexpr size_t pc = (offsetof(Scene, primRight) - offsetof(Scene, camPos)) / 4;
+                    const f3 right = mk3(cam[pc], cam[pc + 1], cam[pc + 2]), down = mk3(cam[pc + 3], cam[pc + 4], cam[pc + 5]);
+#endif
+                    const f3 P = TL + u * right + vv * down;
                     v = P - camPos;
                     cn.primary++;
                 }
                 CRT_DENS_MASK(12, gen);
                 CRT_PSTAMP(e1); CRT_PACC(2, p2b, e1);
-                new_ray(gen, s, v, true, camPos, seed, item);
+                new_ray(std::true_type{}, gen, s, v, true, camPos, seed, item);
                 CRT_PSTAMP(e2); CRT_PACC(3, e1, e2);
                 if (ended) {
                     f3 L = miss ? tex_unpack(skyTexel) : ((depth >= sc.depthLimit) ? mk3(0, 0, 0) : mk3(24, 24, 22));
@@ -480,7 +508,7 @@
 #endif
                 CRT_DENS(14, 1); CRT_DENS(15, n); CRT_DENS_MASK(16, mesh);
                 rec4 s0 = {0, 0, 0, 0}, s1 = s0, s2 = s0, s3 = s0;
-                if (mesh) { const uint32_t so = sc.shadeOff + tri * 64u; s0 = ldg(geom, so); s1 = ldg(geom, so + 16u); s2 = ldg(geom, so + 32u); s3 = ldg(geom, so + 48u); cn.meshhits++; }
+                if (mesh) { const uint32_t so = sc.shadeOff + tri * 64u; s0 = ldp<0>(geom, so); s1 = ldp<1>(geom, so); s2 = ldp<2>(geom, so); s3 = ldp<3>(geom, so); cn.meshhits++; }
                 const bool inside = (meta & kMetaInside) != 0u;
                 const int depth = (int)((meta >> kMetaDepthShift) & 7u);
                 const uint32_t item = meta & kMetaItemMask;
@@ -515,7 +543,7 @@
                             N = normalize3(Nn);
                         } else {
                             const uint32_t io = sc.instOff + (uint32_t)(obj - 2) * 128u + 64u;
-                            const rec4 r0 = ldg(geom, io), r1 = ldg(geom, io + 16), r2 = ldg(geom, io + 32);
+                            const rec4 r0 = ldp<0>(geom, io), r1 = ldp<1>(geom, io), r2 = ldp<2>(geom, io);
                             N = normalize3(mk3(r0.x * Nn.x + r0.y * Nn.y + r0.z * Nn.z + r0.w * 0.0f,
                                                r1.x * Nn.x + r1.y * Nn.y + r1.z * Nn.z + r1.w * 0.0f,
                                                r2.x * Nn.x + r2.y * Nn.y + r2.z * Nn.z + r2.w * 0.0f));
@@ -542,7 +570,7 @@
                         if (cost2 > 0) {
                             const float a = n1 - n2, b2 = n1 + n2, R0 = (a * a) / (b2 * b2), cc = 1 - cosi;
                             const float Fr = R0 + (1 - R0) * (cc * cc * cc * cc * cc);
-                            const f3 T = eta * D + ((eta * cosi - __builtin_sqrtf(__builtin_fabsf(cost2))) * N);
+                            const f3 T = eta * D + ((eta * cosi - sqrt_exact(__builtin_fabsf(cost2))) * N);
                             if (rnd(seed) > Fr) { v = T; newInside = !inside; }
                         }
                     } else {
@@ -562,7 +590,7 @@
                         pre = medium * brdf * 2.0f * CRT_PI;
                     } else pre = c * medium;
                     CRT_PSTAMP(b2); CRT_PACC(6, b1, b2);
-                    const float inv = rcp_exact(__builtin_sqrtf(dot3(v, v)));
+                    const float inv = rcp_exact(sqrt_exact(dot3(v, v)));
                     const f3 nv = norm ? v * inv : v;
                     v = nv;
                     const f3 factor = diffuse ? pre * dot3(nv, N) : pre;
@@ -574,7 +602,7 @@
                     CRT_PSTAMP(b3); CRT_PACC(7, b2, b3);
                 }
                 CRT_PSTAMP(b4);
-                new_ray(act, s, v, false, O, seed, item | ((uint32_t)(depth + 1) << kMetaDepthShift) | (newInside ? kMetaInside : 0u));
+                new_ray(std::false_type{}, act, s, v, false, O, seed, item | ((uint32_t)(depth + 1) << kMetaDepthShift) | (newInside ? kMetaInside : 0u));
 #ifdef CRT_POOL_STAMPS
                 { CRT_PSTAMP(b5); CRT_PACC(8, b4, b5); pst[11]++; }
 #endif
```
